# Yelp/nrtsearch

Measured on AMD Instinct MI355X. Metric: queries/sec, 10M-doc 5-term BM25 top-1000, higher is better.
Workload: dtype f32

## Files before the change

### include/nrtgpu_dev.h

```cpp
#ifndef NRTGPU_DEV_H
#define NRTGPU_DEV_H
#include "nrtgpu.h"
#ifdef __cplusplus
extern "C" {
#endif
int  nrtgpu_bench_closed_loop(nrtgpu_ctx* ctx, const nrtgpu_seg* const* segs, const int32_t* doc_bases, int32_t n_segs,
                              const nrtgpu_bm25_query* queries, int32_t n_queries, int32_t clients, int32_t duration_ms,
                              double* out4);
int  nrtgpu_debug_hold_coalescers(nrtgpu_ctx* ctx, int32_t hold);
int  nrtgpu_debug_coalescer_pending(nrtgpu_ctx* ctx, int32_t which);
int  nrtgpu_debug_dist_inject(nrtgpu_ctx* ctx, int32_t step, int32_t failed_query);
int64_t nrtgpu_debug_live_segments(nrtgpu_ctx* ctx);
int  nrtgpu_debug_spec_counters(nrtgpu_ctx* ctx, int64_t* out3);
int  nrtgpu_debug_term_lookup(const nrtgpu_seg* seg, int32_t field_id, int64_t term_hash, int32_t* kind, int32_t* shift, int64_t* bytes);
int  nrtgpu_debug_knn_bounds(int32_t sim, int32_t dim, double q_norm2, double q_l1, float q_absmax, double nv_max, double nv_min,
                             float rows_absmax, float score_boost, double m, double s, double* out10);

#define NRTGPU_FLAG_PROFILE (7 << 8)
int  nrtgpu_get_scan_profile(nrtgpu_ctx* ctx, double* out16);
int  nrtgpu_get_maxscore_profile(nrtgpu_ctx* ctx, double* out16);
int  nrtgpu_debug_maxscore_meetings(nrtgpu_ctx* ctx, int64_t* out4);
int  nrtgpu_debug_wave_kth(const uint64_t* keys, int32_t n, int32_t r, uint64_t* out);
int64_t nrtgpu_get_maxscore_item_walls(nrtgpu_ctx* ctx, uint64_t* out, int64_t cap_slots, int64_t* n_items);

#ifdef __cplusplus
}
#endif
#endif
```

### nrtsearch_amd/_lib.py

```python
from __future__ import annotations

import ctypes as C
import os

_HERE = os.path.dirname(os.path.abspath(__file__))
LIB_PATH = os.environ.get("NRTGPU_LIB_PATH") or os.path.join(_HERE, "libnrtgpu.so")

NRTGPU_OK = 0
NRTGPU_ERR_INVALID_ARG = -1
NRTGPU_ERR_HIP = -2
NRTGPU_ERR_OOM = -3
NRTGPU_ERR_UNSUPPORTED = -4
NRTGPU_ERR_STATE = -5
NRTGPU_ERR_TIMEOUT = -6
NRTGPU_MAX_K = 1024
NRTGPU_MAX_TERMS = 32
NRTGPU_TILE_DOCS = 1024
NRTGPU_FLAG_NO_PREFETCH = 1
NRTGPU_FLAG_NO_FIXED_POINT = 2
NRTGPU_FLAG_NO_MASK_VARIANT = 4
NRTGPU_FLAG_NO_LIVE_FOLD = 8
NRTGPU_FLAG_NO_PRUNE = 16
NRTGPU_FLAG_PACKED_POSTINGS = 32
NRTGPU_FLAG_BLOCKING_WAIT = 64
NRTGPU_FLAG_NO_VECTOR_SKETCH = 128
NRTGPU_FLAG_PROFILE = 7 << 8
NRTGPU_MAX_MASKS = 8

ABI_SYMBOLS = [
    "nrtgpu_version", "nrtgpu_last_error", "nrtgpu_create", "nrtgpu_destroy",
    "nrtgpu_segment_begin", "nrtgpu_segment_add_field_norms", "nrtgpu_segment_add_terms",
    "nrtgpu_segment_add_vectors", "nrtgpu_segment_seal", "nrtgpu_segment_set_live_docs",
    "nrtgpu_segment_set_mask", "nrtgpu_segment_release", "nrtgpu_segment_device_bytes",
    "nrtgpu_search_bm25", "nrtgpu_search_bm25_batch", "nrtgpu_search_bm25_batch_device",
    "nrtgpu_search_bm25_batch_device_epoch", "nrtgpu_exchange_open", "nrtgpu_exchange_close",
    "nrtgpu_search_bm25_coalesced", "nrtgpu_set_coalescing", "nrtgpu_query_supported",
    "nrtgpu_merge_topk_device", "nrtgpu_knn_exact", "nrtgpu_knn_exact_coalesced", "nrtgpu_knn_search", "nrtgpu_rescore_vectors", "nrtgpu_search_hybrid_batch",
    "nrtgpu_int_to_byte4", "nrtgpu_byte4_to_int", "nrtgpu_bm25_idf", "nrtgpu_bm25_avgdl",
    "nrtgpu_bm25_norm_cache", "nrtgpu_slices", "nrtgpu_plan_item_counts", "nrtgpu_fixed_point_scale", "nrtgpu_get_stats", "nrtgpu_reset_stats",
    "nrtgpu_set_slicing",
    "nrtgpu_blend", "nrtgpu_dist_unique_id", "nrtgpu_dist_init", "nrtgpu_dist_search_bm25_batch", "nrtgpu_dist_allgather_merge", "nrtgpu_segment_fork",
    "nrtgpu_search_bm25_batch_device_begin", "nrtgpu_pending_wait", "nrtgpu_set_thread_deadline_ns", "nrtgpu_monotonic_ns", "nrtgpu_last_diagnostics", "nrtgpu_dist_close", "nrtgpu_dist_owned_range", "nrtgpu_dist_search_bm25_batch_mode", "nrtgpu_dist_exchange_merge", "nrtgpu_dist_exchange_merge_checked", "nrtgpu_search_bm25_shard_device_begin", "nrtgpu_note_shard_speculation", "nrtgpu_dist_knn_exact", "nrtgpu_dist_search_hybrid_batch",
    "nrtgpu_knn_exact_relation", "nrtgpu_set_speculation", "nrtgpu_set_shard_share", "nrtgpu_set_thread_slices",
    "nrtgpu_segment_add_byte_vectors", "nrtgpu_knn_exact_bytes", "nrtgpu_knn_search_bytes", "nrtgpu_byte_vector_score",
    "nrtgpu_rescore_byte_vectors", "nrtgpu_search_hybrid_bytes_batch", "nrtgpu_set_knn_gather",
]
DEV_SYMBOLS = [
    "nrtgpu_bench_closed_loop", "nrtgpu_debug_hold_coalescers", "nrtgpu_debug_coalescer_pending", "nrtgpu_debug_live_segments",
    "nrtgpu_debug_spec_counters", "nrtgpu_get_scan_profile", "nrtgpu_get_maxscore_profile", "nrtgpu_get_maxscore_item_walls",
    "nrtgpu_debug_dist_inject", "nrtgpu_debug_term_lookup", "nrtgpu_debug_knn_bounds",
    "nrtgpu_debug_maxscore_meetings", "nrtgpu_debug_wave_kth",
]
DEV_LIB_PATH = os.path.join(_HERE, "libnrtgpu_dev.so")


class Config(C.Structure):
    _fields_ = [("device_id", C.c_int32), ("max_batch", C.c_int32), ("target_items", C.c_int32),
                ("collect_timing", C.c_int32), ("flags", C.c_int32), ("host_threads", C.c_int32),
                ("lookup_budget_pct", C.c_int32), ("reserved", C.c_int32)]


class Term(C.Structure):
    _fields_ = [("field_id", C.c_int32), ("cache_slot", C.c_int32), ("term_hash", C.c_int64),
                ("weight", C.c_float), ("occur", C.c_int32)]


class Bm25Query(C.Structure):
    _fields_ = [("n_terms", C.c_int32), ("terms", C.POINTER(Term)), ("n_caches", C.c_int32),
                ("norm_cache", C.POINTER(C.c_float)), ("k", C.c_int32), ("total_hits_threshold", C.c_int32),
                ("has_after", C.c_int32), ("after_doc", C.c_int32), ("after_score", C.c_float),
                ("min_should_match", C.c_int32), ("min_competitive_score", C.c_float), ("filter_mask", C.c_int32),
                ("must_not_mask", C.c_int32), ("disjunction_max", C.c_int32),
                ("n_more_filters", C.c_int32), ("more_filters", C.POINTER(C.c_int32)),
                ("n_more_must_not", C.c_int32), ("more_must_not", C.POINTER(C.c_int32)),
                ("tie_breaker", C.c_float), ("reserved", C.c_int32)]


class TopDocs(C.Structure):
    _fields_ = [("n_hits", C.c_int32), ("capacity", C.c_int32), ("docs", C.POINTER(C.c_int32)),
                ("scores", C.POINTER(C.c_float)), ("total_hits", C.c_int64),
                ("total_hits_is_lower_bound", C.c_int32)]


class Diagnostics(C.Structure):
    _fields_ = [("total_ms", C.c_double), ("plan_ms", C.c_double), ("queue_ms", C.c_double), ("device_ms", C.c_double),
                ("postings", C.c_int64), ("queries", C.c_int32), ("items_maxscore", C.c_int32), ("items_scan", C.c_int32),
                ("reserved", C.c_int32)]


class Stats(C.Structure):
    _fields_ = [("batches", C.c_int64), ("queries", C.c_int64), ("scan_launches", C.c_int64),
                ("scan_ms", C.c_double), ("scan_postings", C.c_int64), ("scan_items", C.c_int64),
                ("merge_ms", C.c_double), ("host_plan_ms", C.c_double), ("fixed_point_launches", C.c_int64),
                ("maxscore_launches", C.c_int64), ("maxscore_ms", C.c_double), ("maxscore_postings", C.c_int64),
                ("maxscore_items", C.c_int64), ("knn_panels", C.c_int64), ("knn_score_launches", C.c_int64),
                ("knn_score_ms", C.c_double), ("knn_rows", C.c_int64), ("knn_second_passes", C.c_int64), ("knn_sketch_launches", C.c_int64),
                ("spec_queries", C.c_int64), ("spec_reruns", C.c_int64), ("spec_disabled", C.c_int64), ("spec_scattered", C.c_int64)]


class NrtGpuError(RuntimeError):
    def __init__(self, code: int, message: str):
        super().__init__(f"nrtgpu error {code}: {message}")
        self.code = code


_lib = None
_dev = None


def load() -> C.CDLL:
    global _lib
    if _lib is None:
        _lib = _open(LIB_PATH)
    return _lib


def load_dev() -> C.CDLL:
    global _dev
    if _dev is None:
        _dev = _open(DEV_LIB_PATH)
    return _dev


def _open(path: str) -> C.CDLL:
    if not os.path.exists(path):
        raise ImportError(
            f"{path} is missing: build it with `python -m nrtsearch_amd.build` "
            "(hipcc, gfx950). There is no Python/CPU fallback for the query path.")
    L = C.CDLL(path)
    vp, i32, i64, f32 = C.c_void_p, C.c_int32, C.c_int64, C.c_float
    L.nrtgpu_version.restype = C.c_char_p
    L.nrtgpu_last_error.restype = C.c_char_p
    L.nrtgpu_create.argtypes = [C.POINTER(Config), C.POINTER(vp)]
    L.nrtgpu_destroy.argtypes = [vp]
    L.nrtgpu_destroy.restype = None
    L.nrtgpu_segment_begin.argtypes = [vp, i32, i32, C.POINTER(vp)]
    L.nrtgpu_segment_add_field_norms.argtypes = [vp, i32, vp]
    L.nrtgpu_segment_add_terms.argtypes = [vp, i32, i64, vp, vp, vp, vp]
    L.nrtgpu_segment_add_vectors.argtypes = [vp, i32, i32, i32, vp, vp]
    L.nrtgpu_segment_seal.argtypes = [vp]
    L.nrtgpu_segment_set_live_docs.argtypes = [vp, vp, i32]
    L.nrtgpu_segment_set_mask.argtypes = [vp, i32, vp, i32]
    L.nrtgpu_segment_release.argtypes = [vp]
    L.nrtgpu_segment_release.restype = None
    L.nrtgpu_segment_device_bytes.argtypes = [vp]
    L.nrtgpu_segment_device_bytes.restype = i64
    L.nrtgpu_search_bm25.argtypes = [vp, vp, vp, i32, C.POINTER(Bm25Query), C.POINTER(TopDocs)]
    L.nrtgpu_search_bm25_batch.argtypes = [vp, vp, vp, i32, C.POINTER(Bm25Query), i32, C.POINTER(TopDocs)]
    L.nrtgpu_search_bm25_batch_device.argtypes = [vp, vp, vp, i32, C.POINTER(Bm25Query), i32, i32, vp, vp, vp]
    L.nrtgpu_search_bm25_batch_device_epoch.argtypes = [vp, vp, vp, i32, C.POINTER(Bm25Query), i32, i32, vp, vp, vp, i64]
    L.nrtgpu_search_bm25_coalesced.argtypes = [vp, vp, vp, i32, C.POINTER(Bm25Query), C.POINTER(TopDocs)]
    L.nrtgpu_set_coalescing.argtypes = [vp, i32]
    if hasattr(L, "nrtgpu_bench_closed_loop"):
        L.nrtgpu_bench_closed_loop.argtypes = [vp, vp, vp, i32, C.POINTER(Bm25Query), i32, i32, i32, vp]
    L.nrtgpu_query_supported.argtypes = [vp, vp, i32, C.POINTER(Bm25Query)]
    L.nrtgpu_exchange_open.argtypes = [vp, C.c_char_p, i32, i32]
    L.nrtgpu_exchange_close.argtypes = [vp]
    L.nrtgpu_exchange_close.restype = None
    L.nrtgpu_merge_topk_device.argtypes = [vp, i32, i32, i32, vp, vp, vp, vp, vp, C.POINTER(TopDocs)]
    L.nrtgpu_knn_exact.argtypes = [vp, vp, vp, i32, i32, i32, vp, i32, i32, i32, f32, C.POINTER(TopDocs)]
    L.nrtgpu_knn_exact_coalesced.argtypes = [vp, vp, vp, i32, i32, i32, vp, i32, i32, f32, C.POINTER(TopDocs)]
    L.nrtgpu_knn_exact_coalesced.restype = i32
    L.nrtgpu_knn_search.argtypes = [vp, vp, vp, i32, i32, i32, vp, i32, i32, i32, f32, i32, f32, C.POINTER(TopDocs)]
    L.nrtgpu_segment_add_byte_vectors.argtypes = [vp, i32, i32, i32, vp, vp]
    L.nrtgpu_knn_exact_bytes.argtypes = [vp, vp, vp, i32, i32, i32, vp, i32, i32, i32, f32, C.POINTER(TopDocs)]
    L.nrtgpu_knn_search_bytes.argtypes = [vp, vp, vp, i32, i32, i32, vp, i32, i32, i32, f32, i32, f32, C.POINTER(TopDocs)]
    L.nrtgpu_byte_vector_score.argtypes = [i32, i32, i32, i32, i32, vp]
    L.nrtgpu_set_knn_gather.argtypes = [vp, i32]
    L.nrtgpu_rescore_vectors.argtypes = [vp, vp, vp, i32, i32, i32, vp, i32, f32, vp, vp, i32, C.c_double, C.c_double, i32,
                                         C.POINTER(TopDocs)]
    L.nrtgpu_search_hybrid_batch.argtypes = [vp, vp, vp, i32, C.POINTER(Bm25Query), i32, i32, i32, vp, i32, f32,
                                             C.c_double, C.c_double, i32, C.POINTER(TopDocs)]
    L.nrtgpu_rescore_byte_vectors.argtypes = L.nrtgpu_rescore_vectors.argtypes
    L.nrtgpu_search_hybrid_bytes_batch.argtypes = L.nrtgpu_search_hybrid_batch.argtypes
    L.nrtgpu_int_to_byte4.argtypes = [i32]
    L.nrtgpu_byte4_to_int.argtypes = [i32]
    L.nrtgpu_bm25_idf.argtypes = [i64, i64]
    L.nrtgpu_bm25_idf.restype = f32
    L.nrtgpu_bm25_avgdl.argtypes = [i64, i64]
    L.nrtgpu_bm25_avgdl.restype = f32
    L.nrtgpu_bm25_norm_cache.argtypes = [f32, f32, f32, vp]
    L.nrtgpu_bm25_norm_cache.restype = None
    L.nrtgpu_plan_item_counts.argtypes = [i32, vp, i32, vp]
    L.nrtgpu_fixed_point_scale.argtypes = [f32, vp, i32, vp]
    L.nrtgpu_slices.argtypes = [i32, vp, vp, vp, i32, i32, i32, vp, vp]
    L.nrtgpu_get_stats.argtypes = [vp, C.POINTER(Stats)]
    L.nrtgpu_reset_stats.argtypes = [vp]
    L.nrtgpu_set_thread_slices.argtypes = [vp, i32]
    L.nrtgpu_set_speculation.argtypes = [vp, C.c_float]
    L.nrtgpu_set_speculation.restype = C.c_int
    L.nrtgpu_set_shard_share.argtypes = [vp, C.c_int64, C.c_int64]
    L.nrtgpu_set_shard_share.restype = C.c_int
    L.nrtgpu_knn_exact_relation.argtypes = [vp, vp, vp, C.c_int32, C.c_int32, C.c_int32, C.c_int32]
    L.nrtgpu_reset_stats.restype = None
    if hasattr(L, "nrtgpu_debug_hold_coalescers"):
        L.nrtgpu_debug_hold_coalescers.argtypes = [vp, C.c_int32]
        L.nrtgpu_debug_live_segments.argtypes = [vp]
        L.nrtgpu_debug_live_segments.restype = C.c_int64
        L.nrtgpu_debug_spec_counters.argtypes = [vp, vp]
        L.nrtgpu_debug_spec_counters.restype = C.c_int
        L.nrtgpu_get_maxscore_item_walls.argtypes = [vp, vp, C.c_int64, C.POINTER(C.c_int64)]
        L.nrtgpu_get_maxscore_item_walls.restype = C.c_int64
        L.nrtgpu_debug_coalescer_pending.argtypes = [vp, C.c_int32]
        L.nrtgpu_debug_dist_inject.argtypes = [vp, C.c_int32, C.c_int32]
        L.nrtgpu_get_scan_profile.argtypes = [vp, vp]
        L.nrtgpu_get_maxscore_profile.argtypes = [vp, vp]
        L.nrtgpu_debug_term_lookup.argtypes = [vp, i32, i64, C.POINTER(i32), C.POINTER(i32), C.POINTER(i64)]
    if hasattr(L, "nrtgpu_debug_maxscore_meetings"):
        L.nrtgpu_debug_maxscore_meetings.argtypes = [vp, vp]
        L.nrtgpu_debug_wave_kth.argtypes = [vp, i32, i32, vp]
    if hasattr(L, "nrtgpu_debug_knn_bounds"):
        L.nrtgpu_debug_knn_bounds.argtypes = [i32, i32, C.c_double, C.c_double, f32, C.c_double, C.c_double, f32, f32, C.c_double, C.c_double, vp]
    L.nrtgpu_set_slicing.argtypes = [vp, i32, i32, i32]
    L.nrtgpu_blend.argtypes = [i32, vp, vp, vp, vp, i32, i32, i32, i32, C.POINTER(TopDocs)]
    L.nrtgpu_dist_unique_id.argtypes = [vp]
    L.nrtgpu_dist_init.argtypes = [vp, i32, i32, vp]
    L.nrtgpu_dist_search_bm25_batch.argtypes = [vp, vp, vp, i32, C.POINTER(Bm25Query), i32, C.POINTER(TopDocs)]
    L.nrtgpu_dist_allgather_merge.argtypes = [vp, i32, i32, vp, vp, vp, vp, vp, C.POINTER(TopDocs)]
    L.nrtgpu_segment_fork.argtypes = [vp, vp, i32, C.POINTER(vp)]
    L.nrtgpu_search_bm25_batch_device_begin.argtypes = [vp, vp, vp, i32, C.POINTER(Bm25Query), i32, i32, vp, vp, vp, C.c_int64, vp]
    L.nrtgpu_pending_wait.argtypes = [vp]
    L.nrtgpu_set_thread_deadline_ns.argtypes = [C.c_int64]
    L.nrtgpu_set_thread_deadline_ns.restype = None
    L.nrtgpu_monotonic_ns.argtypes = []
    L.nrtgpu_monotonic_ns.restype = C.c_int64
    L.nrtgpu_last_diagnostics.argtypes = [vp]
    L.nrtgpu_dist_owned_range.argtypes = [vp, i32, i32, vp, vp]
    L.nrtgpu_dist_search_bm25_batch_mode.argtypes = [vp, vp, vp, i32, C.POINTER(Bm25Query), i32, i32, C.POINTER(TopDocs)]
    L.nrtgpu_dist_exchange_merge.argtypes = [vp, i32, i32, vp, vp, vp, vp, vp, i32, C.POINTER(TopDocs)]
    L.nrtgpu_dist_exchange_merge_checked.argtypes = [vp, i32, i32, vp, vp, vp, vp, vp, vp, i32, C.POINTER(TopDocs), vp, vp]
    L.nrtgpu_search_bm25_shard_device_begin.argtypes = [vp, vp, vp, i32, C.POINTER(Bm25Query), i32, i32, vp, vp, vp, i32, vp, vp]
    L.nrtgpu_note_shard_speculation.argtypes = [vp, vp, i32, i32, i32]
    L.nrtgpu_dist_knn_exact.argtypes = [vp, vp, vp, i32, i32, i32, vp, i32, i32, i32, C.c_float, i32, C.POINTER(TopDocs)]
    L.nrtgpu_dist_search_hybrid_batch.argtypes = [vp, vp, vp, i32, C.POINTER(Bm25Query), i32, i32, i32, vp, i32, C.c_float, C.c_double, C.c_double,
                                                  i32, i32, C.POINTER(TopDocs)]
    L.nrtgpu_dist_close.argtypes = [vp]
    L.nrtgpu_dist_close.restype = None
    return L


def check(rc: int) -> None:
    if rc != NRTGPU_OK:
        raise NrtGpuError(rc, load().nrtgpu_last_error().decode("utf-8", "replace"))
```

### nrtsearch_amd/api.py

```python
from __future__ import annotations

import ctypes as C
import dataclasses
import os
import threading
from typing import Dict, List, Optional, Sequence, Tuple, Union

import numpy as np

from . import _lib
from ._lib import NrtGpuError

INT_MAX = 2**31 - 1
TOTAL_HITS_THRESHOLD = 1000


EXCHANGE_ALLGATHER, EXCHANGE_ALLTOALL = 0, 1
EXCHANGE_NO_SPECULATION = 0x100


@dataclasses.dataclass(frozen=True)
class TermQuery:
    field: int
    term: int
# ... 441 lines not shown
    def __init__(self, ctx: GpuContext, leaves: Sequence[GpuSegment], stats: IndexStatistics,
                 similarity: Optional[BM25Similarity] = None):
        self.ctx, self.leaves, self.stats = ctx, list(leaves), stats
        self.similarity = similarity or BM25Similarity()
        n = len(self.leaves)
        self._segs = (C.c_void_p * max(n, 1))(*[l._h for l in self.leaves])
        self._bases = (C.c_int32 * max(n, 1))(*[l.doc_base for l in self.leaves])
        self._cache_memo: Dict[int, np.ndarray] = {}

    def _norm_cache(self, field: int) -> np.ndarray:
        c = self._cache_memo.get(field)
        if c is None:
            c = self.similarity.norm_cache(self.stats.fields[field])
            self._cache_memo[field] = c
        return c

    def _marshal(self, queries: Sequence[Query], managers: Sequence[TopScoreDocCollectorManager]) -> _Marshalled:
        m = _Marshalled(len(queries))
        for qi, (query, mgr) in enumerate(zip(queries, managers)):
            clauses, msm, filters, must_nots, dis_max, tie_breaker = _flatten(query)
            fields: List[int] = []
            terms = (_lib.Term * len(clauses))()
            for ti, (field, term, boost, occur) in enumerate(clauses):
                if field not in self.stats.fields:
                    raise UnsupportedQuery(f"no statistics for field {field}")
                if field not in fields:
                    fields.append(field)
                df = self.stats.doc_freq.get((field, term), 0)
                cs = self.stats.fields[field]
                w = np.float32(np.float32(boost) * self.similarity.idf(df, cs.doc_count)) if df > 0 else np.float32(0)
                terms[ti] = _lib.Term(field, fields.index(field), term, float(w), int(occur))
            cache = np.concatenate([self._norm_cache(f) for f in fields]).astype(np.float32)
            m.keep += [terms, cache]
            q = m.queries[qi]
            q.n_terms = len(clauses)
            q.terms = terms
            q.n_caches = len(fields)
            q.norm_cache = cache.ctypes.data_as(C.POINTER(C.c_float))
            q.k = int(mgr.num_hits)
            q.total_hits_threshold = int(mgr.total_hits_threshold)
            q.has_after = int(mgr.after is not None)
            q.after_doc = int(mgr.after.doc) if mgr.after is not None else 0
            q.after_score = float(mgr.after.score) if mgr.after is not None else 0.0
            q.min_should_match = int(msm)
            q.min_competitive_score = float(mgr.min_competitive_score)
            q.filter_mask = int(filters[0]) if filters else 0
            q.must_not_mask = int(must_nots[0]) if must_nots else 0
            q.disjunction_max = int(dis_max)
            q.tie_breaker = float(np.float32(tie_breaker))
            for ids, n_name, p_name in ((filters[1:], "n_more_filters", "more_filters"), (must_nots[1:], "n_more_must_not", "more_must_not")):
                if ids:
                    arr = (C.c_int32 * len(ids))(*[int(x) for x in ids])
                    m.keep.append(arr)
                    setattr(q, n_name, len(ids))
                    setattr(q, p_name, arr)
        return m

    def search_batch(self, queries: Sequence[Query], managers: Sequence[TopScoreDocCollectorManager]) -> List[TopDocs]:
        n = len(queries)
        m = self._marshal(queries, managers)
        outs = (_lib.TopDocs * n)()
        bufs = []
        for qi, mgr in enumerate(managers):
            cap = max(int(mgr.num_hits), 1)
            d = np.zeros(cap, dtype=np.int32)
            s = np.zeros(cap, dtype=np.float32)
            bufs.append((d, s))
            outs[qi].capacity = cap
            outs[qi].docs = d.ctypes.data_as(C.POINTER(C.c_int32))
            outs[qi].scores = s.ctypes.data_as(C.POINTER(C.c_float))
        _lib.check(_lib.load().nrtgpu_search_bm25_batch(self.ctx._h, self._segs, self._bases, len(self.leaves),
                                                        m.queries, n, outs))
        res = []
        for qi in range(n):
            nh = outs[qi].n_hits
            d, s = bufs[qi]
            res.append(TopDocs(d[:nh].copy(), s[:nh].copy(), int(outs[qi].total_hits),
                               bool(outs[qi].total_hits_is_lower_bound)))
        return res

    def search(self, query: Query, manager: TopScoreDocCollectorManager) -> TopDocs:
        return self.search_batch([query], [manager])[0]

    def dist_search_batch(self, queries: Sequence[Query], managers: Sequence[TopScoreDocCollectorManager],
                          mode: int = EXCHANGE_ALLGATHER) -> List[Optional[TopDocs]]:
        n = len(queries)
        m = self._marshal(queries, managers)
        outs = (_lib.TopDocs * n)()
        bufs = []
        for qi, mgr in enumerate(managers):
            cap = max(int(mgr.num_hits), 1)
            d = np.zeros(cap, dtype=np.int32)
            s = np.zeros(cap, dtype=np.float32)
            bufs.append((d, s))
            outs[qi].capacity = cap
            outs[qi].docs = d.ctypes.data_as(C.POINTER(C.c_int32))
            outs[qi].scores = s.ctypes.data_as(C.POINTER(C.c_float))
        _lib.check(_lib.load().nrtgpu_dist_search_bm25_batch_mode(self.ctx._h, self._segs, self._bases, len(self.leaves), m.queries, n,
                                                                  int(mode), outs))
        return [None if outs[qi].total_hits < 0 else
                TopDocs(bufs[qi][0][: outs[qi].n_hits].copy(), bufs[qi][1][: outs[qi].n_hits].copy(), int(outs[qi].total_hits),
                        bool(outs[qi].total_hits_is_lower_bound)) for qi in range(n)]

    def dist_knn_exact(self, field: int, similarity: str, queries: np.ndarray, k: int, boost: float = 1.0,
                       mode: int = EXCHANGE_ALLGATHER) -> List[Optional[TopDocs]]:
        queries = np.ascontiguousarray(np.atleast_2d(queries), dtype=np.float32)
        if similarity == "normalized_cosine":
            queries = np.ascontiguousarray(queries / np.linalg.norm(queries, axis=1, keepdims=True).astype(np.float32), dtype=np.float32)
        nq, dim = queries.shape
        outs, docs, scores = _topdocs_outputs(nq, int(k))
        _lib.check(_lib.load().nrtgpu_dist_knn_exact(self.ctx._h, self._segs, self._bases, len(self.leaves), int(field),
                                                     self.SIMILARITY[similarity], queries.ctypes.data, nq, dim, int(k),
                                                     C.c_float(boost), int(mode), outs))
        return _topdocs_lists(outs, docs, scores, nq, none_if_negative=True)

    def supported(self, query: Query, manager: TopScoreDocCollectorManager) -> bool:
        m = self._marshal([query], [manager])
        rc = _lib.load().nrtgpu_query_supported(self.ctx._h, self._segs, len(self.leaves), m.queries)
        if rc == _lib.NRTGPU_OK:
            return True
        if rc == _lib.NRTGPU_ERR_UNSUPPORTED:
            return False
        _lib.check(rc)
        return False

    def search_coalesced(self, query: Query, manager: TopScoreDocCollectorManager) -> TopDocs:
        m = self._marshal([query], [manager])
        cap = max(int(manager.num_hits), 1)
        d = np.zeros(cap, dtype=np.int32)
        s = np.zeros(cap, dtype=np.float32)
        out = _lib.TopDocs()
        out.capacity = cap
        out.docs = d.ctypes.data_as(C.POINTER(C.c_int32))
        out.scores = s.ctypes.data_as(C.POINTER(C.c_float))
        _lib.check(_lib.load().nrtgpu_search_bm25_coalesced(self.ctx._h, self._segs, self._bases, len(self.leaves),
                                                            m.queries, C.byref(out)))
        return TopDocs(d[: out.n_hits].copy(), s[: out.n_hits].copy(), int(out.total_hits), bool(out.total_hits_is_lower_bound))

    SIMILARITY = {"cosine": 0, "dot_product": 1, "normalized_cosine": 1, "l2_norm": 2, "max_inner_product": 3}

    def knn_exact(self, field: int, similarity: str, queries: np.ndarray, k: int, boost: float = 1.0) -> List[TopDocs]:
        queries = np.ascontiguousarray(np.atleast_2d(queries), dtype=np.float32)
        if similarity == "normalized_cosine":
            queries = queries / np.linalg.norm(queries, axis=1, keepdims=True).astype(np.float32)
            queries = np.ascontiguousarray(queries, dtype=np.float32)
        nq, dim = queries.shape
        outs, docs, scores = _topdocs_outputs(nq, int(k))
        _lib.check(_lib.load().nrtgpu_knn_exact(self.ctx._h, self._segs, self._bases, len(self.leaves), int(field),
                                                self.SIMILARITY[similarity], queries.ctypes.data, nq, dim, int(k),
                                                C.c_float(boost), outs))
        return _topdocs_lists(outs, docs, scores, nq)

    def knn_exact_coalesced(self, field: int, similarity: str, query: np.ndarray, k: int, boost: float = 1.0) -> TopDocs:
        query = np.ascontiguousarray(query, dtype=np.float32).reshape(-1)
        if similarity == "normalized_cosine":
            query = np.ascontiguousarray(query / np.linalg.norm(query).astype(np.float32), dtype=np.float32)
        out = _lib.TopDocs()
        docs = np.zeros(k, dtype=np.int32)
        scores = np.zeros(k, dtype=np.float32)
        out.capacity = k
        out.docs = docs.ctypes.data_as(C.POINTER(C.c_int32))
        out.scores = scores.ctypes.data_as(C.POINTER(C.c_float))
        _lib.check(_lib.load().nrtgpu_knn_exact_coalesced(self.ctx._h, self._segs, self._bases, len(self.leaves), int(field),
                                                          self.SIMILARITY[similarity], query.ctypes.data, int(query.shape[0]), int(k),
                                                          C.c_float(boost), C.byref(out)))
        return TopDocs(docs[: out.n_hits].copy(), scores[: out.n_hits].copy(), int(out.total_hits), bool(out.total_hits_is_lower_bound))
# ... 198 lines not shown
        self.scores = np.zeros((self.n, kmax), dtype=np.float32)
        for qi in range(self.n):
            self._outs[qi].capacity = kmax
            self._outs[qi].docs = self.docs[qi].ctypes.data_as(C.POINTER(C.c_int32))
            self._outs[qi].scores = self.scores[qi].ctypes.data_as(C.POINTER(C.c_float))

    def run(self, d_keys: int, d_counts: int, d_hits: int) -> None:
        _lib.check(_lib.load().nrtgpu_merge_topk_device(
            self.ctx._h, self.n_lists, self.n, self.k_stride, C.c_void_p(d_keys), C.c_void_p(d_counts),
            C.c_void_p(d_hits), self._ks.ctypes.data, self._thr.ctypes.data, self._outs))

    def run_dist(self, d_keys: int, d_counts: int, d_hits: int, mode: int = EXCHANGE_ALLGATHER) -> None:
        _lib.check(_lib.load().nrtgpu_dist_exchange_merge(
            self.ctx._h, self.n, self.k_stride, C.c_void_p(d_keys), C.c_void_p(d_counts), C.c_void_p(d_hits),
            self._ks.ctypes.data, self._thr.ctypes.data, int(mode), self._outs))

    def run_dist_checked(self, d_keys: int, d_counts: int, d_hits: int, d_guess: int, mode: int = EXCHANGE_ALLGATHER) -> np.ndarray:
        failed = np.zeros(self.n, dtype=np.uint8)
        n_failed = C.c_int32(0)
        _lib.check(_lib.load().nrtgpu_dist_exchange_merge_checked(
            self.ctx._h, self.n, self.k_stride, C.c_void_p(d_keys), C.c_void_p(d_counts), C.c_void_p(d_hits), C.c_void_p(d_guess),
            self._ks.ctypes.data, self._thr.ctypes.data, int(mode), self._outs, failed.ctypes.data, C.byref(n_failed)))
        return np.flatnonzero(failed) if n_failed.value else np.zeros(0, dtype=np.int64)

    def kth_keys(self) -> np.ndarray:
        n_hits = np.frombuffer(self._outs, dtype=np.int32).reshape(self.n, C.sizeof(_lib.TopDocs) // 4)[:, 0]
        rows = np.arange(self.n)
        col = self._ks.astype(np.int64) - 1
        keys = (self.scores.view(np.uint32)[rows, col].astype(np.uint64) << np.uint64(32)) | (np.uint64(0xFFFFFFFF) - self.docs[rows, col].astype(np.uint64))
        return np.where(n_hits >= self._ks, keys, np.uint64(0))

    def owned(self, qi: int) -> bool:
        return self._outs[qi].total_hits >= 0

    def topdocs(self, qi: int) -> TopDocs:
        o = self._outs[qi]
        return TopDocs(self.docs[qi, : o.n_hits].copy(), self.scores[qi, : o.n_hits].copy(), int(o.total_hits),
                       bool(o.total_hits_is_lower_bound))


def merge_topk_device(ctx: GpuContext, n_lists: int, n_queries: int, k_stride: int, d_keys: int, d_counts: int,
                      d_hits: int, ks: Sequence[int], thresholds: Sequence[int]) -> List[TopDocs]:
    pm = PreparedMerge(ctx, n_lists, n_queries, k_stride, ks, thresholds)
    pm.run(d_keys, d_counts, d_hits)
    return [pm.topdocs(qi) for qi in range(n_queries)]


def slices(max_docs: Sequence[int], num_docs: Optional[Sequence[int]] = None, virtual_shards: int = 1,
           slice_max_docs: int = 250_000, slice_max_segments: int = 5):
    n = len(max_docs)
    md = np.ascontiguousarray(max_docs, dtype=np.int32)
    nd = np.ascontiguousarray(num_docs if num_docs is not None else max_docs, dtype=np.int32)
    sl = np.full(max(n, 1), -1, dtype=np.int32)
    sh = np.full(max(n, 1), -1, dtype=np.int32)
    ns = _lib.load().nrtgpu_slices(n, md.ctypes.data, nd.ctypes.data, None, int(virtual_shards), int(slice_max_docs),
                                   int(slice_max_segments), sl.ctypes.data, sh.ctypes.data)
    if ns < 0:
        _lib.check(ns)
    out: List[List[int]] = [[] for _ in range(ns)]
    for i in range(n):
        out[sl[i]].append(i)
    return out, sh[:n].tolist()


def debug_knn_bounds(sim: int, dim: int, q_norm2: float, q_l1: float, q_absmax: float, nv_max: float, nv_min: float,
                     rows_absmax: float, score_boost: float = 1.0, m: float = 0.0, s: float = 0.0) -> dict:
    out = np.zeros(10, dtype=np.float64)
    _lib.check(_lib.load().nrtgpu_debug_knn_bounds(int(sim), int(dim), float(q_norm2), float(q_l1), C.c_float(q_absmax), float(nv_max),
                                                   float(nv_min), C.c_float(rows_absmax), C.c_float(score_boost), float(m), float(s),
                                                   out.ctypes.data))
    names = ("e32", "e16", "result_upper32", "result_upper16", "estimate_lower32", "estimate_lower16", "q_scale", "rows_scale")
    d = {n: float(out[i]) for i, n in enumerate(names)}
    d["q_scale_usable"], d["rows_scale_usable"] = bool(out[8]), bool(out[9])
    return d


def debug_wave_kth(keys: np.ndarray, r: int) -> int:
    keys = np.ascontiguousarray(keys, dtype=np.uint64)
    out = np.zeros(1, dtype=np.uint64)
    _lib.check(_lib.load().nrtgpu_debug_wave_kth(keys.ctypes.data, len(keys), int(r), out.ctypes.data))
    return int(out[0])


def blend(retriever_docs: Sequence[np.ndarray], retriever_scores: Optional[Sequence[np.ndarray]] = None,
          boosts: Optional[Sequence[float]] = None, mode: str = "rrf", k: int = 60, start_hit: int = 0, top_hits: int = 10) -> TopDocs:
    n = len(retriever_docs)
    docs = [np.ascontiguousarray(d, dtype=np.int32) for d in retriever_docs]
    scs = [np.ascontiguousarray(s_, dtype=np.float32) for s_ in retriever_scores] if retriever_scores is not None else None
    dp = (C.c_void_p * max(n, 1))(*[d.ctypes.data for d in docs])
    sp = (C.c_void_p * max(n, 1))(*[s_.ctypes.data for s_ in scs]) if scs is not None else None
    counts = np.asarray([len(d) for d in docs], dtype=np.int32)
    b = np.ascontiguousarray(boosts, dtype=np.float32) if boosts is not None else None
    cap = max(int(top_hits), 1)
    od, os_ = np.zeros(cap, np.int32), np.zeros(cap, np.float32)
    out = _lib.TopDocs()
    out.capacity = cap
    out.docs = od.ctypes.data_as(C.POINTER(C.c_int32))
    out.scores = os_.ctypes.data_as(C.POINTER(C.c_float))
    _lib.check(_lib.load().nrtgpu_blend(n, dp, sp, counts.ctypes.data, b.ctypes.data if b is not None else None,
                                        0 if mode == "rrf" else 1, int(k), int(start_hit), int(top_hits), C.byref(out)))
    return TopDocs(od[: out.n_hits].copy(), os_[: out.n_hits].copy(), int(out.total_hits), bool(out.total_hits_is_lower_bound))


def weighted_rrf_blend(retriever_hits: Sequence[np.ndarray], boosts: Optional[Sequence[float]] = None, k: int = 60,
                       start_hit: int = 0, top_hits: int = 10) -> TopDocs:
    if k < 1:
        raise ValueError(f"k must be >= 1, got: {k}")
    if top_hits == 0 or start_hit > top_hits:
        return TopDocs(np.zeros(0, np.int32), np.zeros(0, np.float32), 0, True)
    merged: Dict[int, np.float32] = {}
    for ri, docs in enumerate(retriever_hits):
        w = np.float32(1.0 if boosts is None else boosts[ri])
        for i, doc in enumerate(np.asarray(docs).tolist()):
            contrib = np.float32(w / np.float32(k + i + 1))
            merged[doc] = np.float32(merged[doc] + contrib) if doc in merged else contrib
    order = sorted(merged.items(), key=lambda kv: (-float(kv[1]), kv[0]))[: min(top_hits, len(merged))]
    page = order[min(start_hit, len(order)):]
    return TopDocs(np.asarray([d for d, _ in page], np.int32), np.asarray([s for _, s in page], np.float32),
                   len(merged), True)
```

### nrtsearch_amd/csrc/devtools.cpp

```cpp
#include "runtime_internal.h"
#include "../../include/nrtgpu_dev.h"

extern "C" int nrtgpu_bench_closed_loop(nrtgpu_ctx* ctx, const nrtgpu_seg* const* segs, const int32_t* doc_bases,
                                        int32_t n_segs, const nrtgpu_bm25_query* queries, int32_t n_queries,
                                        int32_t clients, int32_t duration_ms, double* out4) {
  if (!ctx || !queries || !out4 || n_queries <= 0 || clients <= 0 || duration_ms <= 0)
    return fail(NRTGPU_ERR_INVALID_ARG, "bad closed-loop arguments");
  std::vector<std::vector<float>> lat((size_t)clients);
  std::vector<int> rcs((size_t)clients, 0);
  std::vector<std::string> errs((size_t)clients);
  const auto t_begin = std::chrono::steady_clock::now();
  const auto t_stop = t_begin + std::chrono::milliseconds(duration_ms);
  auto client = [&](int c) {
    int32_t kmax = 1;
    for (int i = 0; i < n_queries; ++i) kmax = std::max(kmax, queries[i].k);
    std::vector<int32_t> docs((size_t)kmax);
    std::vector<float> scores((size_t)kmax);
    size_t i = (size_t)c * 7919u;
    for (;;) {
      const auto t0 = std::chrono::steady_clock::now();
      if (t0 >= t_stop) break;
      nrtgpu_topdocs o{};
      o.capacity = kmax;
      o.docs = docs.data();
      o.scores = scores.data();
      const int rc = nrtgpu_search_bm25_coalesced(ctx, segs, doc_bases, n_segs, &queries[i % (size_t)n_queries], &o);
      if (rc != 0) {
        rcs[(size_t)c] = rc;
        errs[(size_t)c] = g_last_error;
        break;
      }
      lat[(size_t)c].push_back(std::chrono::duration<float, std::milli>(std::chrono::steady_clock::now() - t0).count());
      ++i;
    }
  };
  std::vector<std::thread> pool;
  for (int c = 0; c < clients; ++c) pool.emplace_back(client, c);
  for (auto& t : pool) t.join();
  const double secs = std::chrono::duration<double>(std::chrono::steady_clock::now() - t_begin).count();
  for (int c = 0; c < clients; ++c)
    if (rcs[(size_t)c] != 0) return fail(rcs[(size_t)c], "client %d: %s", c, errs[(size_t)c].c_str());
  std::vector<float> all;
  for (auto& v : lat) all.insert(all.end(), v.begin(), v.end());
  std::sort(all.begin(), all.end());
  out4[0] = (double)all.size();
  out4[1] = secs;
  out4[2] = all.empty() ? 0.0 : all[all.size() / 2];
  out4[3] = all.empty() ? 0.0 : all[(size_t)((double)all.size() * 0.99)];
  return NRTGPU_OK;
}


extern "C" int nrtgpu_debug_knn_bounds(int32_t sim, int32_t dim, double q_norm2, double q_l1, float q_absmax, double nv_max, double nv_min,
                                       float rows_absmax, float score_boost, double m, double s, double* out10) {
  if (!out10 || sim < 0 || sim > 3 || dim <= 0 || (dim & 15)) return fail(NRTGPU_ERR_INVALID_ARG, "bad knn_bounds arguments");
  float q_scale = 1.0f, rows_scale = 1.0f;
  const bool q_ok = hostmath::knn_sketch_scale(q_absmax, &q_scale), rows_ok = hostmath::knn_sketch_scale(rows_absmax, &rows_scale);
  const double e_rel = (double)hostmath::knn_e_rel(), b = (double)score_boost;
  const float e32 = hostmath::knn_bound32(sim, dim, q_norm2, nv_max, b);
  const float e16 = hostmath::knn_bound16(sim, dim, q_norm2, q_l1, 1.0 / (double)q_scale, nv_max, nv_min, 1.0 / (double)rows_scale, b);
  out10[0] = (double)e32;
  out10[1] = (double)e16;
  out10[2] = knn_result_upper(sim, m, (double)e32, e_rel, b);
  out10[3] = knn_result_upper(sim, m, (double)e16, e_rel, b);
  out10[4] = knn_estimate_lower(sim, s, (double)e32, e_rel, b);
  out10[5] = knn_estimate_lower(sim, s, (double)e16, e_rel, b);
  out10[6] = (double)q_scale;
  out10[7] = (double)rows_scale;
  out10[8] = q_ok ? 1.0 : 0.0;
  out10[9] = rows_ok ? 1.0 : 0.0;
  return NRTGPU_OK;
}

extern "C" int nrtgpu_debug_maxscore_meetings(nrtgpu_ctx* ctx, int64_t* out4) {
  if (!ctx || !out4) return fail(NRTGPU_ERR_INVALID_ARG, "NULL argument");
  std::lock_guard<std::mutex> lk(ctx->stats_mu);
  for (int i = 0; i < 4; ++i) out4[i] = ctx->ms_meetings[i];
  return NRTGPU_OK;
}

extern "C" int nrtgpu_debug_wave_kth(const uint64_t* keys, int32_t n, int32_t r, uint64_t* out) {
  if (!keys || !out || n < 1 || n > kMsCandCap || r < 1 || r > n) return fail(NRTGPU_ERR_INVALID_ARG, "bad wave_kth arguments (1 <= r <= n <= %d)", kMsCandCap);
  uint64_t* d = nullptr;
  if (hipMalloc((void**)&d, ((size_t)n + 1) * sizeof(uint64_t)) != hipSuccess) return fail(NRTGPU_ERR_OOM, "hipMalloc");
  hipError_t e = hipMemcpy(d, keys, (size_t)n * sizeof(uint64_t), hipMemcpyHostToDevice);
  if (e == hipSuccess) {
    launch_debug_wave_kth(nullptr, d, (uint32_t)n, (uint32_t)r, d + n);
    e = hipGetLastError();
  }
  if (e == hipSuccess) e = hipMemcpy(out, d + n, sizeof(uint64_t), hipMemcpyDeviceToHost);
  (void)hipFree(d);
  if (e != hipSuccess) return fail(NRTGPU_ERR_HIP, "wave_kth: %s", hipGetErrorString(e));
  return NRTGPU_OK;
}
```

### nrtsearch_amd/csrc/kernels.hip

```cpp
#include <hip/hip_runtime.h>
#include <stdint.h>

#include "bm25_common.hiph"

namespace nrtgpu {

struct ScanSmem {
  uint64_t acc[kScanWaves][kTileDocs];
  uint64_t cand[kCandCap];
  uint32_t tab[kTabTerms][kTabEntries];
  float    cache[kLdsCaches][256];
  alignas(16) uint32_t w_incl[kScanWaves][kMaxTerms];
  alignas(16) uint32_t w_rec[kScanWaves][kMaxTerms][4];
  uint32_t w_before[kScanWaves][kMaxTerms];
  TopkScratch sc;
  uint64_t theta;
  uint64_t thr;
  uint32_t cnt;
  uint32_t tile_cand;
  uint32_t slot_hits[kSliceSlots];
  uint32_t slot_slice[kSliceSlots];
  uint32_t rz_flag;
  uint32_t cnt_valid;
  uint32_t next_tile;
// ... 848 lines not shown
  }
}

__global__ __launch_bounds__(256)
void apply_live_kernel(const uint32_t* __restrict__ docids, uint32_t* __restrict__ fnorm, uint64_t n,
                       const uint64_t* __restrict__ live) {
  const uint64_t stride = (uint64_t)gridDim.x * blockDim.x;
  for (uint64_t p = (uint64_t)blockIdx.x * blockDim.x + threadIdx.x; p < n; p += stride) {
    uint32_t c = fnorm[p];
    const bool esc = (c >> 31) != 0u;
    if (esc) c &= ~0x40000000u;
    else if ((c >> 20) != 0u) c = (((c >> 20) & 15u) << 9) | (c & 0x1FCu);
    bool is_live = true;
    if (live) {
      const uint32_t d = docids[p];
      is_live = (live[d >> 6] >> (d & 63u)) & 1ull;
    }
    if (!is_live) c = esc ? (c | 0x40000000u) : ((((c >> 9) & 15u) << 20) | (c & 0x1FCu));
    fnorm[p] = c;
  }
}

__global__ __launch_bounds__(256)
void pack_count_kernel(const uint32_t* __restrict__ fnorm, uint64_t n, uint32_t* __restrict__ counts) {
  __shared__ uint32_t total;
  if (threadIdx.x == 0) total = 0;
  __syncthreads();
  const uint64_t p0 = (uint64_t)blockIdx.x << kPackEscBlockShift;
  uint32_t mine = 0;
  for (uint32_t i = threadIdx.x; i < (1u << kPackEscBlockShift); i += 256u) {
    const uint64_t p = p0 + i;
    if (p < n && (fnorm[p] >> 31) != 0u) ++mine;
  }
  if (mine) atomicAdd(&total, mine);
  __syncthreads();
  if (threadIdx.x == 0) counts[blockIdx.x] = total;
}

__global__ __launch_bounds__(256)
void pack_write_kernel(const uint32_t* __restrict__ docids, const uint32_t* __restrict__ fnorm, uint64_t n,
                       const uint32_t* __restrict__ dir, uint32_t* __restrict__ exceptions, uint32_t* __restrict__ packed) {
  __shared__ uint32_t wave_cnt[8][4];
  const uint32_t lane = threadIdx.x & 63u, wave = threadIdx.x >> 6;
  const uint64_t p0 = (uint64_t)blockIdx.x << kPackEscBlockShift;
  uint32_t c[8];
  unsigned long long ball[8];
#pragma unroll
  for (int r = 0; r < 8; ++r) {
    const uint64_t p = p0 + (uint64_t)r * 256u + threadIdx.x;
    c[r] = p < n ? fnorm[p] : 0u;
    ball[r] = __builtin_amdgcn_ballot_w64((c[r] >> 31) != 0u);
    if (lane == 0) wave_cnt[r][wave] = (uint32_t)__popcll(ball[r]);
  }
  __syncthreads();
  const uint32_t e_block = dir[blockIdx.x];
#pragma unroll
  for (int r = 0; r < 8; ++r) {
    const uint64_t p = p0 + (uint64_t)r * 256u + threadIdx.x;
    if (p >= n) continue;
    uint32_t code = c[r] >> 2;
    if ((c[r] >> 31) != 0u) {
      uint32_t before = 0;
      for (int rr = 0; rr < 8; ++rr)
        for (int ww = 0; ww < 4; ++ww)
          if (rr < r || (rr == r && (uint32_t)ww < wave)) before += wave_cnt[rr][ww];
      const uint32_t e = e_block + before + (uint32_t)__popcll(ball[r] & ((1ull << lane) - 1ull));
      exceptions[e] = c[r];
      code = kPackEscBase + (e & kPackEscLowMask);
    }
    packed[p] = ((docids[p] & kPackDocMask) << kPackCodeBits) | code;
  }
}

__global__ __launch_bounds__(256)
void expand_terms_kernel(const DQExpand* __restrict__ qx, const DQTerm* __restrict__ qterms, const uint32_t* __restrict__ out_begin,
                         uint32_t n_queries, uint32_t n_leaves, DTerm* __restrict__ out) {
  const uint32_t i = blockIdx.x * blockDim.x + threadIdx.x;
  if (i >= n_queries * n_leaves) return;
  const uint32_t ob = out_begin[i];
  if (ob == 0xFFFFFFFFu) return;
  const uint32_t q = i / n_leaves, leaf = i - q * n_leaves;
  const DQExpand x = qx[q];
  const DQTerm* const qt = qterms + x.term_begin;
  for (uint32_t t = 0; t < x.n_terms; ++t) {
    DTerm d = qt[t].table[leaf];
    if (d.docids == nullptr) continue;
    const uint32_t cnt = __float_as_uint(d.weight);
    const float w = qt[t].weight;
    uint32_t rank = 0;
    for (uint32_t u = 0; u < x.n_terms; ++u) {
      if (u == t) continue;
      const DTerm& o = qt[u].table[leaf];
      if (o.docids == nullptr) continue;
      const uint32_t oc = __float_as_uint(o.weight);
      const float ow = qt[u].weight;
      const bool before = x.by_weight ? (ow > w || (ow == w && (oc < cnt || (oc == cnt && u < t))))
                                      : (oc > cnt || (oc == cnt && u < t));
      rank += before ? 1u : 0u;
    }
    d.weight = w;
    d.cache_slot = qt[t].cache_slot;
    d.tab_slot = qt[t].tab_slot;
    d.fx_scale = qt[t].fx_scale;
    d.fx_shift = qt[t].fx_shift;
    out[ob + rank] = d;
  }
}
void launch_expand_terms(hipStream_t stream, const DQExpand* qx, const DQTerm* qterms, const uint32_t* out_begin, uint32_t n_queries,
                         uint32_t n_leaves, DTerm* out) {
  const uint64_t n = (uint64_t)n_queries * n_leaves;
  if (n == 0) return;
  hipLaunchKernelGGL(expand_terms_kernel, dim3((uint32_t)((n + 255) / 256)), dim3(256), 0, stream, qx, qterms, out_begin, n_queries,
                     n_leaves, out);
}

__global__ __launch_bounds__(256)
void slice_relation_kernel(const uint32_t* __restrict__ slice_sum, const DQuery* __restrict__ queries, uint32_t n_slices,
                           uint64_t* __restrict__ out_hits, uint32_t n) {
  const uint32_t q = blockIdx.x * blockDim.x + threadIdx.x;
  if (q >= n) return;
  if ((out_hits[q] >> 48) != 0ull) return;
  const uint32_t floor_ = queries[q].gte_floor;
  if (floor_ == 0xFFFFFFFFu) return;
  const uint32_t* sums = slice_sum + queries[q].slice_base;
  bool gte = false;
  for (uint32_t i = 0; i < n_slices; ++i) gte = gte || sums[i] > floor_;
  if (gte) out_hits[q] += kHitsPrunedUnit;
}
void launch_slice_relation(hipStream_t stream, const uint32_t* slice_sum, const DQuery* queries, uint32_t n_slices, uint64_t* out_hits,
                           uint32_t n) {
  if (n == 0) return;
  hipLaunchKernelGGL(slice_relation_kernel, dim3((n + 255) / 256), dim3(256), 0, stream, slice_sum, queries, n_slices, out_hits, n);
}

__global__ __launch_bounds__(256)
void patch_hits_kernel(const uint64_t* __restrict__ lower, uint64_t* __restrict__ hits, uint32_t n) {
  const uint32_t q = blockIdx.x * blockDim.x + threadIdx.x;
  if (q < n && lower[q] != 0ull && (hits[q] >> 48) != 0ull) hits[q] = kHitsPrunedUnit + lower[q] + (hits[q] & kHitsSpecInvalid);
}
void launch_patch_hits(hipStream_t stream, const uint64_t* lower, uint64_t* hits, uint32_t n) {
  if (n == 0) return;
  hipLaunchKernelGGL(patch_hits_kernel, dim3((n + 255) / 256), dim3(256), 0, stream, lower, hits, n);
}

void launch_pack_count(hipStream_t stream, const uint32_t* fnorm, uint64_t n, uint32_t n_blocks, uint32_t* counts) {
  if (n_blocks == 0) return;
  hipLaunchKernelGGL(pack_count_kernel, dim3(n_blocks), dim3(256), 0, stream, fnorm, n, counts);
}
void launch_pack_write(hipStream_t stream, const uint32_t* docids, const uint32_t* fnorm, uint64_t n, uint32_t n_blocks,
                       const uint32_t* dir, uint32_t* exceptions, uint32_t* packed) {
  if (n_blocks == 0) return;
  hipLaunchKernelGGL(pack_write_kernel, dim3(n_blocks), dim3(256), 0, stream, docids, fnorm, n, dir, exceptions, packed);
}
void launch_apply_live(hipStream_t stream, const uint32_t* docids, uint32_t* fnorm, uint64_t n, const uint64_t* live) {
  if (n == 0) return;
  const uint64_t blocks = (n + 1023) / 1024;
  hipLaunchKernelGGL(apply_live_kernel, dim3((uint32_t)(blocks < 8192 ? blocks : 8192)), dim3(256), 0, stream, docids, fnorm, n, live);
}
void launch_bm25_scan(hipStream_t stream, bool fixed_point, bool pipelined, bool packed, int ablation, uint32_t n_items, const DItem* items,
                      const DPart* parts, const DTerm* terms, const DQuery* queries, const float* caches, unsigned long long* theta_g,
                      unsigned long long* quant_g, const DExchange* xch, uint32_t* slice_sum, uint64_t* item_keys, uint32_t* item_counts,
                      uint64_t* item_hits, uint32_t k_stride, uint64_t* item_prof) {
  if (n_items == 0) return;
#define NRT_LAUNCH_K(F, P, A, K)                                                                                  \
  hipLaunchKernelGGL((bm25_scan_kernel<F, P, A, K>), dim3(n_items), dim3(kScanThreads), 0, stream, items, parts, terms, queries, \
                     caches, theta_g, quant_g, xch, slice_sum, item_keys, item_counts, item_hits, k_stride, item_prof)
#define NRT_LAUNCH(F, P, A)                 \
  do {                                      \
    if (packed) NRT_LAUNCH_K(F, P, A, true);  \
    else NRT_LAUNCH_K(F, P, A, false);      \
  } while (0)
#define NRT_LAUNCH_FX(P, A)            \
  do {                                 \
    if (fixed_point) NRT_LAUNCH(true, P, A); \
    else NRT_LAUNCH(false, P, A);      \
  } while (0)
  if (ablation == 8) { NRT_LAUNCH(true, true, 8); return; }
  if (ablation == 9) { NRT_LAUNCH_FX(true, 9); return; }
  if (!pipelined) { NRT_LAUNCH_FX(false, 0); return; }
  switch (ablation) {
#ifdef NRTGPU_DEV
    case 1: NRT_LAUNCH_K(false, true, 1, false); break;
    case 2: NRT_LAUNCH_K(false, true, 2, false); break;
    case 3: NRT_LAUNCH_K(false, true, 3, false); break;
    case 4: NRT_LAUNCH_K(false, true, 4, false); break;
    case 6: NRT_LAUNCH_K(false, true, 6, false); break;
    case 7: NRT_LAUNCH_FX(true, 7); break;
#endif
    default: NRT_LAUNCH_FX(true, 0); break;
  }
#undef NRT_LAUNCH_FX
#undef NRT_LAUNCH
#undef NRT_LAUNCH_K
}

void launch_merge_topk(hipStream_t stream, uint32_t n_queries, const uint64_t* in_keys, const uint32_t* in_counts,
                       const uint64_t* in_hits, const uint32_t* list_idx, const uint32_t* q_base,
// ... 19 lines not shown
```

### nrtsearch_amd/csrc/maxscore.hip

```cpp
#include <hip/hip_runtime.h>
#include <stdint.h>

#include "bm25_common.hiph"

namespace nrtgpu {

constexpr int kMsWinWords = kMsWinDocs / 32;
constexpr int kSl = kMsSlots;
typedef uint32_t u32x2 __attribute__((ext_vector_type(2)));
typedef const NRT_GLOBAL u32x2* gvec2_ptr;

struct alignas(16) WClause {
  uint64_t docids, fnorm;
  uint64_t begin;
  uint32_t count, pad0;
  float    weight;
  int32_t  fx_scale;
  uint32_t flags;
  uint32_t pad;
  uint64_t u_after;
  uint64_t look;
  uint64_t cells, start;
};
static_assert(sizeof(WClause) == 80, "WClause layout");
// ... 144 lines not shown
    if (guess > s.theta) {
      s.theta = guess;
      s.thr = acc_threshold<true>(guess, fx_E);
      atomicMax(theta_g, (unsigned long long)guess);
      atomicMax(s.spec_slot, (unsigned long long)guess);
    }
    const uint32_t ws = s.wins_started;
    s.spec_at = ws >= s.q_wins ? 0u : max(ws * s.spec_grow16 / 16u, ws + (uint32_t)kMsWaves);
  }
  __syncthreads();
  if (tid == 0) s.rz_flag = 0;
  __syncthreads();
}

__device__ __forceinline__ bool ms_meet(MsSmem& s, uint32_t k, int fx_E, unsigned long long* theta_g, const DExchange* xch = nullptr,
                                        uint32_t query = 0) {
  __syncthreads();
  if (!__hip_atomic_load(&s.rz_flag, __ATOMIC_RELAXED, __HIP_MEMORY_SCOPE_WORKGROUP)) return false;
  ms_compact((__attribute__((address_space(3))) MsSmem*)&s, k, fx_E, theta_g, xch, query);
  return true;
}

__device__ __noinline__ void ms_estimate(__attribute__((address_space(3))) MsSmem* sp, uint32_t k, int fx_E,
                                         unsigned long long* theta_g, const DExchange* xch) {
  MsSmem& s = *(MsSmem*)sp;
  const uint32_t lane = threadIdx.x & 63u;
  const uint32_t ws = (uint32_t)__builtin_amdgcn_readfirstlane((int)__hip_atomic_load(&s.wins_started, __ATOMIC_RELAXED, __HIP_MEMORY_SCOPE_WORKGROUP));
  const uint32_t at = (uint32_t)__builtin_amdgcn_readfirstlane((int)__hip_atomic_load(&s.spec_at, __ATOMIC_RELAXED, __HIP_MEMORY_SCOPE_WORKGROUP));
  const uint32_t n = (uint32_t)__builtin_amdgcn_readfirstlane((int)__hip_atomic_load(&s.cnt, __ATOMIC_RELAXED, __HIP_MEMORY_SCOPE_WORKGROUP));
  if (at != 0u && ws >= at && n <= (uint32_t)kMsCandCap) {
    const bool exchanging = xch && xch->world > 1u;
    uint32_t r = 0;
    if (s.spec_z16 != 0u && !exchanging && __hip_atomic_load(&s.prune_on, __ATOMIC_RELAXED, __HIP_MEMORY_SCOPE_WORKGROUP) != 0u) {
      const float m = (float)k * fminf(1.0f, (float)ws / (float)max(s.q_wins, 1u));
      const float rr = m + (float)s.spec_z16 * (1.0f / 16.0f) * sqrtf(m) + 2.0f;
      r = rr < (float)k ? (uint32_t)rr : 0u;
    }
    uint64_t guess = 0;
    if (r != 0u && n > r) guess = topk_kth_wave(s.cand, n, r, &s.sc);
    if (lane == 0u) {
      if (guess > s.theta) {
        __hip_atomic_store(&s.theta, guess, __ATOMIC_RELAXED, __HIP_MEMORY_SCOPE_WORKGROUP);
        __hip_atomic_store(&s.thr, acc_threshold<true>(guess, fx_E), __ATOMIC_RELAXED, __HIP_MEMORY_SCOPE_WORKGROUP);
        atomicMax(theta_g, (unsigned long long)guess);
        atomicMax(s.spec_slot, (unsigned long long)guess);
      }
      s.spec_at = ws >= s.q_wins ? 0u : max(ws * s.spec_grow16 / 16u, ws + (uint32_t)kMsWaves);
      s.n_est += 1u;
    }
  }
  wave_lds_phase();
  if (lane == 0u) __hip_atomic_store(&s.spec_busy, 0u, __ATOMIC_RELEASE, __HIP_MEMORY_SCOPE_WORKGROUP);
}

__device__ __forceinline__ bool ms_reserve(MsSmem& s, uint32_t lane, uint32_t mine, uint32_t& pos) {
  const uint32_t incl = scan64_dpp(mine);
  const uint32_t wave_total = (uint32_t)__builtin_amdgcn_readlane((int)incl, 63);
  uint32_t wbase = 0;
  if (lane == 0) {
    wbase = atomicAdd(&s.cnt, wave_total);
    if (wbase + wave_total > (uint32_t)kMsCandCap) {
      if (wbase <= (uint32_t)kMsCandCap) s.cnt_valid = wbase;
      __hip_atomic_store(&s.rz_flag, 1u, __ATOMIC_RELAXED, __HIP_MEMORY_SCOPE_WORKGROUP);
    }
  }
  wbase = (uint32_t)__builtin_amdgcn_readfirstlane((int)wbase);
  pos = wbase + incl - mine;
  return wbase + wave_total <= (uint32_t)kMsCandCap;
}

template <bool PROF, bool PACKED, int SHAPES>
__global__ __launch_bounds__(kMsThreads)
void bm25_maxscore_kernel(const MsArgs* __restrict__ launch) {
  constexpr bool TWO = SHAPES == 2;
  __shared__ MsSmem s;
  const uint32_t tid = threadIdx.x;
  const uint32_t wave = tid >> 6, lane = tid & 63u;
  for (uint32_t round = 0;; ++round) {
    const uint64_t wall_entry = PROF ? wall_clock64() : 0ull;
    const ms_args_ptr ap = ms_fresh(launch);
    const __attribute__((address_space(4))) DHelp& hp = ap->help;
    const DItem* const items = as_global(ap->items);
    const DPart* const parts = as_global(ap->parts);
    const DTerm* const terms = as_global(ap->terms);
    const DExchange* const xch = as_global(ap->xch);
    bool helper = false;
    uint32_t my_item = 0, out_slot = 0;
    {
      const uint32_t min_rem = hp.min_rem & 0xFFFFu;
      const bool greedy = ((hp.min_rem >> 16) & 1u) != 0u;
      for (int attempt = 0; attempt < 2; ++attempt) {
        if (tid == 0) {
          s.pick = 0ull;
          s.role[0] = __hip_atomic_load(hp.item_next, __ATOMIC_RELAXED, __HIP_MEMORY_SCOPE_AGENT);
          s.role[1] = __hip_atomic_load(hp.help_used, __ATOMIC_RELAXED, __HIP_MEMORY_SCOPE_AGENT);
          s.role[2] = 0u;
          s.role[3] = __hip_atomic_load(hp.help_off, __ATOMIC_RELAXED, __HIP_MEMORY_SCOPE_AGENT);
        }
        __syncthreads();
        const uint32_t q_next = s.role[0];
        const bool queue_empty = attempt == 1 || q_next >= hp.n_own;
        const bool slots_left = s.role[1] < hp.n_help;
        if (queue_empty && (!slots_left || s.role[3] != 0u)) return;
        const bool look = slots_left && (queue_empty || (hp.alpha16 != 0u && q_next >= hp.n_cus + hp.n_cus / 4u));
        if (look) {
          const uint64_t now = wall_clock64();
          float t_rem = 0.f;
          if (!queue_empty) {
            uint32_t mine = 0;
            for (uint32_t i = tid; i < hp.n_own; i += kMsThreads) {
              const uint64_t t0 = __hip_atomic_load(hp.item_t0 + i, __ATOMIC_RELAXED, __HIP_MEMORY_SCOPE_AGENT);
              if (t0 == 0ull) continue;
              mine += min(items[i].flags >> 8, (uint32_t)kMsWaves + __hip_atomic_load(hp.win_next + i, __ATOMIC_RELAXED, __HIP_MEMORY_SCOPE_AGENT));
            }
            mine = (uint32_t)__builtin_amdgcn_readlane((int)scan64_dpp(mine), 63);
            if (lane == 0 && mine != 0u) atomicAdd(&s.role[2], mine);
            __syncthreads();
            const uint32_t handed = s.role[2];
            const uint64_t ts = __hip_atomic_load(hp.t_start, __ATOMIC_RELAXED, __HIP_MEMORY_SCOPE_AGENT);
            t_rem = (handed == 0u || ts == 0ull || now <= ts) ? 3.0e38f
                    : (float)(now - ts) * (float)(hp.total_wins > handed ? hp.total_wins - handed : 0u) / (float)handed * ((float)hp.alpha16 * (1.0f / 16.0f));
          }
          for (uint32_t i = tid; i < hp.n_own; i += kMsThreads) {
            const uint32_t fl = items[i].flags;
            if ((fl & 3u) == kMsModeExact) continue;
            const uint32_t nw = fl >> 8;
            const uint32_t taken = (uint32_t)kMsWaves + __hip_atomic_load(hp.win_next + i, __ATOMIC_RELAXED, __HIP_MEMORY_SCOPE_AGENT);
            if (taken + min_rem > nw) continue;
            const uint64_t t0 = __hip_atomic_load(hp.item_t0 + i, __ATOMIC_RELAXED, __HIP_MEMORY_SCOPE_AGENT);
            if (t0 == 0ull || now <= t0) continue;
            const uint32_t hc = __hip_atomic_load(hp.help_cnt + i, __ATOMIC_RELAXED, __HIP_MEMORY_SCOPE_AGENT);
            const float left = (float)(now - t0) * (float)(nw - taken) / ((float)(taken - (uint32_t)kMsWaves + 1u) * (float)(1u + hc));
            if (!queue_empty && !(left > t_rem)) continue;
            uint32_t hsh = ((blockIdx.x + round * gridDim.x) * 0x9E3779B9u) ^ (i * 0x85EBCA6Bu) ^ (uint32_t)now;
            hsh ^= hsh >> 16; hsh *= 0x7FEB352Du; hsh ^= hsh >> 15; hsh *= 0x846CA68Bu; hsh ^= hsh >> 16;
            const float u = ((float)(hsh >> 8) + 0.5f) * (1.0f / 16777216.0f);
            const float key = greedy ? left : left / -__logf(u);
            atomicMax((unsigned long long*)&s.pick, ((unsigned long long)__float_as_uint(key) << 32) | (unsigned long long)(i + 1u));
          }
        }
        __syncthreads();
        if (tid == 0) {
          const uint64_t pick = s.pick;
          uint32_t r_item = 0xFFFFFFFFu, r_slot = 0xFFFFFFFFu;
          if ((uint32_t)pick != 0u) {
            const uint32_t slot = atomicAdd(hp.help_used, 1u);
            if (slot < hp.n_help) {
              r_slot = slot;
              r_item = (uint32_t)pick - 1u;
              atomicAdd(hp.help_cnt + r_item, 1u);
            }
          } else if (queue_empty && look) {
            __hip_atomic_store(hp.help_off, 1u, __ATOMIC_RELAXED, __HIP_MEMORY_SCOPE_AGENT);
          }
          if (r_slot == 0xFFFFFFFFu && !queue_empty) {
            const uint32_t it = atomicAdd(hp.item_next, 1u);
            if (it < hp.n_own) r_item = it;
          }
          s.role[0] = r_item;
          s.role[1] = r_slot;
        }
        __syncthreads();
        const uint32_t r_item = s.role[0], r_slot = s.role[1];
        __syncthreads();
        if (r_item != 0xFFFFFFFFu) {
          my_item = r_item;
          helper = r_slot != 0xFFFFFFFFu;
// ... 32 lines not shown
      const uint64_t theta0 = __hip_atomic_load(my_theta_g, __ATOMIC_RELAXED, __HIP_MEMORY_SCOPE_AGENT);
      s.theta = theta0;
      s.thr = acc_threshold<true>(theta0, fx_E);
      s.cnt = 0;
      s.cnt_valid = 0;
      s.rz_flag = 0;
      s.spec_busy = 0;
      s.n_meet = s.n_over = s.n_est = 0;
      if (!helper) {
        const unsigned long long now0 = (unsigned long long)wall_clock64();
        __hip_atomic_store(hp.item_t0 + my_item, now0, __ATOMIC_RELAXED, __HIP_MEMORY_SCOPE_AGENT);
        if (my_item == 0u) __hip_atomic_store(hp.t_start, now0, __ATOMIC_RELAXED, __HIP_MEMORY_SCOPE_AGENT);
      }
      s.prune_on = mode == kMsModePrune ? 1u : 0u;
      const bool spec = hp.spec_g != nullptr && hp.spec_z16 != 0u;
      s.wins_started = 0;
      s.q_wins = spec ? as_global(ap->q_wins)[item.query] : 0u;
      s.spec_z16 = spec ? hp.spec_z16 : 0u;
      s.spec_slot = spec ? as_global(hp.spec_g) + item.query : nullptr;
      s.spec_at = spec ? max(hp.spec_sched & 255u, 1u) : 0u;
      s.spec_grow16 = max((hp.spec_sched >> 8) & 255u, 17u);
      s.spec_meet = (hp.spec_sched >> 16) & 1u;
      for (int i = 0; i < kSliceSlots; ++i) s.slot_hits[i] = s.slot_slice[i] = 0u;
      for (int i = 0; i < 16; ++i) s.prof[i] = 0;
    }
    const uint64_t t_item0 = PROF ? __builtin_readcyclecounter() : 0ull;
    const uint64_t wall0 = PROF ? wall_clock64() : 0ull;
    uint64_t tc_meet = 0, tc_part = 0, tc_walk = 0;
    __syncthreads();
    if (xch && tid < 64u) {
      const uint64_t pb = exchange_bound(*xch, item.query, 0ull, tid);
      if (tid == 0 && pb > s.theta) {
        s.theta = pb;
        s.thr = acc_threshold<true>(pb, fx_E);
      }
    }
    for (uint32_t slot = 0; slot < item.n_tabs; ++slot) {
      const float w = items[my_item].tab_weight[slot];
      const int scale = items[my_item].tab_scale[slot];
      const float* cache = &s.cache[items[my_item].tab_cache[slot]][0];
      for (uint32_t e = tid; e < (uint32_t)kTabEntries; e += kMsThreads)
        s.tab[slot][e] = e < (uint32_t)kTabNorms ? 0u : score_value<true>(bm25_score(w, (float)(int32_t)(e >> 7), cache[e & 127u]), scale);
    }
    __syncthreads();
  #ifndef NRT_MS_PHASE_CLOCKS
    if (PROF && tid == 0) s.prof[8] = __builtin_readcyclecounter() - t_item0;
  #endif

    uint32_t* const seen = &s.seen[wave][0];
    WClause* const wcl = &s.wc[wave][0];
    const uint32_t wcl_addr = lds_addr(wcl);
    uint32_t wave_hits = 0;
    uint32_t cur_slot = 0;
    uint64_t pc_post = 0, pc_surv = 0, pc_look = 0, pc_cand = 0, pc_chunks = 0, pc_wins = 0;
  #ifdef NRT_MS_PHASE_CLOCKS
    uint64_t ph[9] = {0, 0, 0, 0, 0, 0, 0, 0, 0}, ph_t = 0;
  #endif
  #ifdef NRT_MS_COUNT_ROUNDS
    uint64_t pc_dense = 0, pc_sparse = 0, pc_steps = 0, pc_tas = 0, pc_crounds = 0;
  #endif
    const uint32_t item_wins = item.flags >> 8;
    uint32_t sc_mul = 1u;
    if (ap->scatter != 0u && item_wins > 3u && item_wins < 65536u) {
      const uint32_t primes[4] = {2654435761u, 2246822519u, 3266489917u, 668265263u};
      uint32_t best = 0xFFFFFFFFu;
  #pragma unroll
      for (int i = 0; i < 4; ++i) {
        const uint32_t a = primes[i] % item_wins;
        const uint32_t x = a * 1000u, y = item_wins * 618u;
        const uint32_t dist = x > y ? x - y : y - x;
        if (a > 1u && dist < best) {
          best = dist;
          sc_mul = a;
        }
      }
    }
    auto window_of_take = [&](uint32_t h) -> uint32_t {
      return (sc_mul == 1u || h >= item_wins) ? h : (h * sc_mul) % item_wins;
    };
    uint32_t g = window_of_take(helper ? (uint32_t)kMsWaves + (uint32_t)__builtin_amdgcn_readfirstlane((int)first_win) : wave);
    uint32_t pi = 0;
    uint32_t win_base = 0;

    for (;;) {
      DPart part;
      uint32_t part_wins = 0;
      if (sc_mul != 1u) {
        pi = 0;
        win_base = 0;
      }
      for (;; ++pi) {
        if (pi >= item.n_parts) break;
        part = parts[item.part_begin + pi];
        part_wins = (part.tile_end - (part.tile_begin & ~(win_tiles - 1u)) + win_tiles - 1u) / win_tiles;
        if (g < win_base + part_wins) break;
        win_base += part_wins;
      }
      if (pi >= item.n_parts) break;
      {
        const uint32_t p_slot = part.slice >> 24;
        if (p_slot != cur_slot && wave_hits != 0u) {
          if (lane == 0) atomicAdd(&s.slot_hits[cur_slot], wave_hits);
          wave_hits = 0;
        }
        cur_slot = p_slot;
        if (lane == 0) s.slot_slice[p_slot] = part.slice & 0xFFFFFFu;
      }
      const uint32_t n_terms = part.n_terms;
      const DTerm* const part_terms = terms + part.term_begin;

      uint64_t my_ub = 0, my_suf = 0;
      const uint64_t t_part0 = PROF ? __builtin_readcyclecounter() : 0ull;
      const DTerm mt = part_terms[min(lane, n_terms - 1u)];
      {
        uint32_t ub_raw = 0;
        for (uint32_t pass = 0; pass * 4u < n_terms; ++pass) {
          const uint32_t tt = pass * 4u + (lane >> 4), i = lane & 15u;
          const DTerm* Tp = part_terms + min(tt, n_terms - 1u);
          const DTermAux* ax = Tp->aux;
          const float w = Tp->weight;
          const int scale = Tp->fx_scale;
          const float* cache = &s.cache[Tp->cache_slot][0];
          uint32_t v = 0;
          if (tt < n_terms) {
            if (i < 12u) {
              const uint32_t nb = ax->min_norm[i];
              if (nb != 0xFFu) v = score_value<true>(bm25_score(w, (float)(int32_t)(i + 1u), cache[nb]), scale);
            } else if (i == 12u) {
              const uint32_t mf = ax->esc_max_freq;
              if (mf != 0u) v = score_value<true>(bm25_score(w, (float)(int32_t)mf, cache[ax->esc_min_norm]), scale);
            }
          }
  #pragma unroll
          for (int dlt = 8; dlt > 0; dlt >>= 1) v = max(v, (uint32_t)__shfl_xor((int)v, dlt, 64));
          const uint32_t got = (uint32_t)__shfl((int)v, (int)((lane & 3u) * 16u), 64);
          if ((lane >> 2) == pass) ub_raw = got;
        }
        if (lane < n_terms) my_ub = (uint64_t)ub_raw << mt.fx_shift;
      }
      uint64_t my_after = 0;
      {
        uint64_t run = 0;
        for (int m = (int)n_terms - 1; m >= 0; --m) {
          const uint64_t ub = readlane_u64(my_ub, (uint32_t)m);
          if (lane == (uint32_t)m) my_after = run;
          run = use_max ? max(run, ub) : run + ub;
          if (lane == (uint32_t)m) my_suf = run;
        }
      }
      const gu32_ptr my_cells = (gu32_ptr)mt.cell_off;
      const uint32_t my_shift = mt.shift;
      if (lane < n_terms) {
        WClause w;
        w.docids = (uint64_t)mt.docids;
        w.fnorm = (uint64_t)mt.fnorm;
        w.begin = 0;
        w.count = w.pad0 = 0;
        w.weight = mt.weight;
        w.fx_scale = mt.fx_scale;
        const DTermAux* const ax = mt.aux;
        const uint32_t look_kind = ax->look_kind;
        w.flags = ((mt.tab_slot & 0xFFFFu) < (uint32_t)kTabTerms ? (mt.tab_slot & 0xFFFFu) : 7u) | (TWO && (mt.tab_slot & kTabSlotRequired) ? 8u : 0u) |
                  (mt.fx_shift << 4) | (mt.cache_slot << 8) | ((mt.shift & 31u) << 16) | ((look_kind & 7u) << 24) | (((uint32_t)ax->look_shift & 31u) << 27);
        w.pad = 0;
        w.u_after = my_after;
        w.look = look_kind != kLookNone ? (uint64_t)ax->look : 0ull;
        w.cells = (uint64_t)mt.cell_off;
        w.start = mt.start;
        wcl[lane] = w;
      }
      const uint32_t req_mask = TWO ? (uint32_t)__builtin_amdgcn_ballot_w64(lane < n_terms && (mt.tab_slot & kTabSlotRequired) != 0u) : 0u;
      const uint32_t first_req = req_mask != 0u ? (uint32_t)__builtin_ctz(req_mask) : 0xFFu;
      if (PROF) tc_part += __builtin_readcyclecounter() - t_part0;

      for (;;) {
        const uint64_t t_win0 = PROF ? __builtin_readcyclecounter() : 0ull;
        const uint32_t ta = (part.tile_begin & ~(win_tiles - 1u)) + (g - win_base) * win_tiles;
        const uint32_t t0 = max(ta, part.tile_begin);
        const uint32_t t1 = min(ta + win_tiles, part.tile_end);
        const uint32_t doc_lo = t0 * (uint32_t)kTileDocs;
        const uint32_t doc_span = min(t1 * (uint32_t)kTileDocs, part.max_doc) - doc_lo;
        if (PROF) pc_wins += 1;
        {
          uint32_t est = 0;
          if (lane == 0) {
            const uint32_t ws = atomicAdd(&s.wins_started, 1u) + 1u, at = s.spec_at;
            if (at != 0u && ws >= at) {
              if (s.spec_meet != 0u) __hip_atomic_store(&s.rz_flag, 1u, __ATOMIC_RELAXED, __HIP_MEMORY_SCOPE_WORKGROUP);
              else est = atomicCAS(&s.spec_busy, 0u, 1u) == 0u ? 1u : 0u;
            }
          }
          if (__builtin_amdgcn_readfirstlane((int)est) != 0)
            ms_estimate((__attribute__((address_space(3))) MsSmem*)&s, k, fx_E, my_theta_g, xch);
        }
        uint32_t g_new = 0;
        if (lane == 0) g_new = (uint32_t)kMsWaves + __hip_atomic_fetch_add(win_next_g, 1u, __ATOMIC_RELAXED, __HIP_MEMORY_SCOPE_AGENT);
        uint64_t theta_other = 0, thr_other = 0;
        if (multi_item) {
          theta_other = __hip_atomic_load(my_theta_g, __ATOMIC_RELAXED, __HIP_MEMORY_SCOPE_AGENT);
          thr_other = acc_threshold<true>(theta_other, fx_E);
          if (mode == kMsModeCount && lane == 0 && __hip_atomic_load(my_prune_g, __ATOMIC_RELAXED, __HIP_MEMORY_SCOPE_AGENT) != 0u)
            __hip_atomic_store(&s.prune_on, 1u, __ATOMIC_RELAXED, __HIP_MEMORY_SCOPE_WORKGROUP);
        }
        uint32_t my_lo = 0, my_hi = 0;
        if (lane < n_terms) {
          my_lo = my_cells[t0 >> my_shift];
          my_hi = my_cells[((t1 - 1u) >> my_shift) + 1u];
        }
        if (n_terms > 1u) {
  #pragma unroll
          for (int j = 0; j < kMsWinWords / 64 / 4; ++j) *(u32x4*)&seen[(lane + 64u * (uint32_t)j) * 4u] = u32x4{0u, 0u, 0u, 0u};
        }
        uint32_t ng = 0;
        {
          const uint64_t thr_w = __hip_atomic_load(&s.prune_on, __ATOMIC_RELAXED, __HIP_MEMORY_SCOPE_WORKGROUP) ? loosen(max(s.thr, thr_other)) : 0ull;
          const uint64_t pb = mt.start + my_lo, pe = mt.start + my_hi;
          if (lane < n_terms) {
            if (my_suf >= thr_w && pe > pb && (!SHAPES || msm <= 1u || lane + msm <= n_terms) && (!TWO || lane <= first_req)) ng = (uint32_t)((pe - (pb & ~3ull) + (uint64_t)(kSl - 1)) / (uint64_t)kSl);
            *(u32x4*)&wcl[lane].begin = u32x4{(uint32_t)pb, (uint32_t)(pb >> 32), (uint32_t)(pe - pb), 0u};
          }
        }
        const uint32_t incl = scan32_dpp(ng);
        uint32_t pre[kMsMaxTerms];
  #pragma unroll
        for (int i = 0; i < kMsMaxTerms; ++i) pre[i] = (uint32_t)__builtin_amdgcn_readlane((int)incl, i);
        const uint32_t n_groups = pre[kMsMaxTerms - 1];

  #ifdef NRT_MS_PHASE_CLOCKS
        if (PROF) ph_t = t_win0;
  #endif
        NRT_PH_MARK(0);
        for (uint32_t v0 = 0; v0 < n_groups; v0 += 64u) {
          const uint32_t v = v0 + lane;
          const bool act = v < n_groups;
          uint32_t c = 0, before = 0;
  #pragma unroll
          for (int i = 0; i < kMsMaxTerms - 1; ++i) {
            c += (v >= pre[i]) ? 1u : 0u;
            before = (v >= pre[i]) ? pre[i] : before;
          }
          const uint32_t c_first = (uint32_t)__builtin_amdgcn_readfirstlane((int)c);
          const uint64_t theta = max(s.theta, theta_other), thr = loosen(max(s.thr, thr_other));
          const bool pruning = __hip_atomic_load(&s.prune_on, __ATOMIC_RELAXED, __HIP_MEMORY_SCOPE_WORKGROUP) != 0u;
          const uint64_t thr_p = pruning ? thr : 0ull;
          if (readlane_u64(my_suf, c_first) < thr_p) break;
          if (PROF) pc_chunks += 1;
          const uint32_t rec = wcl_addr + c * (uint32_t)sizeof(WClause);
          const u32x4 r0 = *(const u32x4*)lds_ptr(rec), r1 = *(const u32x4*)lds_ptr(rec + 16u), r2 = *(const u32x4*)lds_ptr(rec + 32u);
          const uint64_t u_after = *(const uint64_t*)lds_ptr(rec + 48u);
          const uint64_t col_d = ((uint64_t)r0[1] << 32) | r0[0], col_c = ((uint64_t)r0[3] << 32) | r0[2];
          const uint64_t p_begin = ((uint64_t)r1[1] << 32) | r1[0];
          const uint32_t flags = r2[2];
          const uint32_t q0 = (v - before) * (uint32_t)kSl;
          const uint64_t mine0 = (p_begin & ~3ull) + (uint64_t)q0;
          uint32_t d[kSl], cd[kSl];
  #pragma unroll
          for (int j = 0; j < kSl; ++j) d[j] = cd[j] = 0u;
          if (act) {
            const u32x4 d0 = __builtin_nontemporal_load((gvec_ptr)(col_d + mine0 * 4u));
            const u32x4 d1 = kSl > 4 ? __builtin_nontemporal_load((gvec_ptr)(col_d + mine0 * 4u) + 1) : d0;
            if (PACKED) {
              const uint32_t sw = doc_lo & ~kPackDocMask;
  #pragma unroll
              for (int j = 0; j < 4; ++j) {
                d[j] = (d0[j] >> kPackCodeBits) | sw;
                cd[j] = (d0[j] & kPackCodeMask) << 2;
                if (kSl > 4) {
                  d[(4 + j) % kSl] = (d1[j] >> kPackCodeBits) | sw;
                  cd[(4 + j) % kSl] = (d1[j] & kPackCodeMask) << 2;
                }
              }
            } else {
              const u32x4 c0 = __builtin_nontemporal_load((gvec_ptr)(col_c + mine0 * 4u));
              const u32x4 c1 = kSl > 4 ? __builtin_nontemporal_load((gvec_ptr)(col_c + mine0 * 4u) + 1) : c0;
  #pragma unroll
              for (int j = 0; j < 4; ++j) {
                d[j] = d0[j];
                cd[j] = c0[j];
                if (kSl > 4) {
                  d[(4 + j) % kSl] = d1[j];
                  cd[(4 + j) % kSl] = c1[j];
                }
              }
            }
          }
          NRT_PH_MARK(1);
          uint32_t vmask = 0;
          {
            const uint32_t rel = q0 - ((uint32_t)p_begin & 3u), cnt = act ? r1[2] : 0u;
  #pragma unroll
            for (int j = 0; j < kSl; ++j)
              if (rel + (uint32_t)j < cnt && d[j] - doc_lo < doc_span) vmask |= 1u << j;
          }
          uint32_t val[kSl];
          {
            const uint32_t tab = flags & 7u;
            const char* tb = (const char*)&s.tab[tab == 7u ? 0u : tab][0];
            uint32_t cor = 0;
  #pragma unroll
// ... 582 lines not shown
```

### nrtsearch_amd/csrc/plan.h

```cpp
#pragma once
#include <math.h>
#include <stdint.h>

namespace nrtgpu {

#ifndef NRT_SCAN_WAVES
#define NRT_SCAN_WAVES 12
#endif
#ifndef NRT_TILE_DOCS
#define NRT_TILE_DOCS 1024
#endif
constexpr int kTileDocs = NRT_TILE_DOCS;
constexpr int kScanWaves = NRT_SCAN_WAVES;
constexpr int kScanThreads = kScanWaves * 64;
static_assert(kScanWaves % 4 == 0 && kTileDocs % 64 == 0 && kTileDocs / 64 <= 16, "scan workgroup shape");
static_assert(kScanWaves * kTileDocs * 8 <= 96 * 1024, "accumulators exceed their LDS share");
constexpr int kCandCap = (kScanWaves == 12) ? 1920 : 1664;
constexpr int kMergeCap = 2048;
constexpr int kLdsCaches = 4;
constexpr int kTabTerms = 5;
constexpr int kTabMaxFreq = 12;
constexpr int kTabNorms = 128;
constexpr int kTabEntries = (kTabMaxFreq + 1) * kTabNorms;
constexpr int kMaxK = 1024;
constexpr int kMaxTerms = 32;
constexpr uint32_t kPackDocBits = 20;
constexpr uint32_t kPackCodeBits = 12;
constexpr uint32_t kPackCodeMask = (1u << kPackCodeBits) - 1u;
constexpr uint32_t kPackDocMask = (1u << kPackDocBits) - 1u;
constexpr uint32_t kPackEscBase = (uint32_t)kTabEntries;
constexpr uint32_t kPackEscBlockShift = 11;
constexpr uint32_t kPackEscLowMask = (1u << kPackEscBlockShift) - 1u;
static_assert(kPackEscBase + kPackEscLowMask < (1u << kPackCodeBits), "exception codes must fit the 12-bit code");
constexpr uint32_t kPackMaxCellShift = kPackDocBits - 10;
static_assert(kTileDocs == 1024 || kPackMaxCellShift > 0, "packed postings assume 1024-doc sub-tiles");

struct DTermAux;
struct alignas(16) DTerm {
  const uint32_t* docids;
  const uint32_t* fnorm;
  const uint32_t* cell_off;
  uint64_t start;
  const DTermAux* aux;
  uint32_t shift;
  float    weight;
  uint32_t cache_slot;
  uint32_t tab_slot;
  int32_t  fx_scale;
  uint32_t fx_shift;
};
static_assert(sizeof(DTerm) == 64, "DTerm layout");

struct alignas(16) DQTerm {
  const DTerm* table;
  float    weight;
  uint32_t cache_slot;
  uint32_t tab_slot;
  int32_t  fx_scale;
  uint32_t fx_shift;
  uint32_t pad;
};
static_assert(sizeof(DQTerm) == 32, "DQTerm layout");
struct alignas(16) DQExpand {
  uint32_t term_begin;
  uint32_t n_terms;
  uint32_t by_weight;
  uint32_t pad;
};
static_assert(sizeof(DQExpand) == 16, "DQExpand layout");

constexpr uint32_t kLookNone = 0, kLookBits = 1, kLookCells = 2;
struct alignas(16) DTermAux {
  const void* look;
  uint8_t  min_norm[12];
  uint8_t  esc_min_norm;
  uint8_t  look_kind;
  uint8_t  look_shift;
  uint8_t  pad;
  uint32_t esc_max_freq;
  uint32_t pad2;
};
static_assert(sizeof(DTermAux) == 32, "DTermAux layout");

#ifndef NRT_MS_WIN_TILES
#define NRT_MS_WIN_TILES 64
#endif
#ifndef NRT_MS_WAVES
#define NRT_MS_WAVES 12
#endif
#ifndef NRT_MS_SLOTS
#define NRT_MS_SLOTS 8
#endif
constexpr int kMsWaves = NRT_MS_WAVES;
constexpr int kMsSlots = NRT_MS_SLOTS;
static_assert(kMsSlots == 4 || kMsSlots == 8, "MaxScore kernel: 4 or 8 postings per lane");
constexpr int kMsThreads = kMsWaves * 64;
static_assert(kMsThreads <= 1024, "a workgroup holds at most 16 waves");
constexpr int kMsWinTiles = NRT_MS_WIN_TILES;
constexpr int kMsWinDocs = kMsWinTiles * kTileDocs;
constexpr int kMsMaxTerms = 8;
constexpr int64_t kMsExactMaxPostings = 1 << 18;
#ifndef NRT_MS_CAND_CAP
#define NRT_MS_CAND_CAP (NRT_MS_WIN_TILES > 32 ? 2304 : 3072)
#endif
constexpr int kMsCandCap = NRT_MS_CAND_CAP;
static_assert(kMsCandCap >= kMaxK + 512, "candidate buffer too small");
constexpr uint64_t kHitsPrunedUnit = 1ull << 48;
constexpr uint64_t kHitsSpecInvalid = 1ull << 47;

struct alignas(16) DPart {
  const uint64_t* live_bits;
  uint32_t term_begin;
  uint32_t n_terms;
  uint32_t tile_begin, tile_end;
  uint32_t max_doc;
  int32_t  doc_base;
  uint32_t tile_offset;
  uint32_t slice;
};
static_assert(sizeof(DPart) == 48, "DPart layout");

struct alignas(16) DItem {
  uint32_t query;
  uint32_t part_begin;
  uint32_t n_parts;
  uint32_t cache_off;
  uint32_t n_caches;
  uint32_t n_tabs;
  float    tab_weight[kTabTerms];
  uint32_t tab_cache[kTabTerms];
  int32_t  tab_scale[kTabTerms];
  int32_t  fx_E;
  uint32_t peer_slot;
  uint32_t flags;
};
static_assert(sizeof(DItem) == 96, "DItem layout");

struct alignas(16) DQuery {
  uint32_t k;
  uint32_t has_after;
  int32_t  after_doc;
  float    after_score;
  uint32_t item_begin;
  uint32_t n_items;
  uint32_t min_should_match;
  uint32_t combine_max;
  uint32_t gte_floor;
  uint32_t slice_base;
  uint32_t sec_mode;
  float    tie_breaker;
};
static_assert(sizeof(DQuery) == 48, "DQuery layout");
constexpr int kSliceSlots = 8;
constexpr uint32_t kMsModePrune = 0, kMsModeExact = 1, kMsModeCount = 2;
constexpr uint32_t kMsSecNone = 0, kMsSecTieBreaker = 1, kMsSecReqOpt = 2;
constexpr uint32_t kTabSlotNone = 0xFFFFu, kTabSlotRequired = 1u << 16;
constexpr int kMsmCountShift = 56;

struct DHelp {
  uint32_t* win_next;
  uint32_t* help_cnt;
  unsigned long long* item_t0;
  uint32_t* help_head;
  uint32_t* help_query;
  uint32_t* help_off;
  uint32_t* item_next;
  uint32_t* help_used;
  unsigned long long* t_start;
  uint32_t n_own, n_help;
  uint32_t slot_base;
  uint32_t min_rem;
  uint32_t total_wins;
  uint32_t alpha16;
  uint32_t n_cus;
  uint32_t persistent;
  unsigned long long* spec_g;
  uint32_t spec_z16, spec_sched;
  unsigned long long* walls;
};

struct DExchange;
struct MsArgs {
  const DItem* items;
  const DPart* parts;
  const DTerm* terms;
  const DQuery* queries;
  const float* caches;
  unsigned long long* theta_g;
  uint32_t* slice_sum;
  uint32_t* q_prune;
  const DExchange* xch;
  uint64_t* item_keys;
  uint32_t* item_counts;
  uint64_t* item_hits;
  uint64_t* item_prof;
  const uint32_t* q_wins;
  uint32_t k_stride;
  uint32_t scatter;
  DHelp help;
};

constexpr int kExchangeSlots = 8;
struct alignas(16) DExchange {
  unsigned long long* slot;
  uint32_t world, rank;
  uint32_t stride;
  uint32_t tag;
};
static_assert(sizeof(DExchange) == 32, "DExchange layout");

struct DVecSeg {
  const float* vecs;
  const float* vnorm2;
  const int32_t* ord_to_doc;
  int32_t doc_base, max_doc, n_vec, pad;
};
static_assert(sizeof(DVecSeg) == 40, "DVecSeg layout");

struct alignas(16) DKnnLeaf {
  const void* sketch;
  const float* vnorm2;
  const int32_t* ord_to_doc;
  const uint64_t* accept;
  int64_t tile_begin;
  int32_t n_rows, doc_base;
  float inv_rows_scale;
  int32_t pad[3];
};
static_assert(sizeof(DKnnLeaf) == 64, "DKnnLeaf layout");

__host__ __device__ inline double knn_result_upper(int sim, double m, double e_abs, double e_rel, double boost) {
  if (sim == 2) {
    if (!(m > 0.0)) return 0.0;
    const double d2 = boost / m - 1.0;
    const double lo = d2 - (e_abs + e_rel * (1.0 + d2));
    return boost / (1.0 + (lo > 0.0 ? lo : 0.0)) * (1.0 + 1e-6);
  }
  return (m + e_abs + e_rel * (m < 0.0 ? -m : m)) * (1.0 + 1e-6);
}
__host__ __device__ inline double knn_estimate_lower(int sim, double s, double e_abs, double e_rel, double boost) {
  if (sim == 2) {
    if (!(s > 0.0)) return 0.0;
    const double d2 = boost / s - 1.0;
    return boost / (1.0 + (d2 > 0.0 ? d2 : 0.0) + e_abs + e_rel * (1.0 + d2)) * (1.0 - 1e-6);
  }
  return (s - (e_abs + e_rel * (s < 0.0 ? -s : s))) * (1.0 - 1e-6);
}

struct alignas(16) DKnnBytesLeaf {
  const void* tiles;
  const int32_t* vnorm2;
  const int32_t* ord_to_doc;
  const uint64_t* accept;
  int64_t tile_begin;
  int32_t n_rows, doc_base;
  int32_t pad[4];
};
static_assert(sizeof(DKnnBytesLeaf) == 64, "DKnnBytesLeaf layout");
struct DByteVecSeg {
  const void* tiles;
  const int32_t* vnorm2;
  const int32_t* ord_to_doc;
  int32_t doc_base, max_doc, n_vec, pad;
};
static_assert(sizeof(DByteVecSeg) == 40, "DByteVecSeg layout");

struct alignas(16) DKnnGatherLeaf {
  const void* rows;
  const int32_t* vnorm2;
  const int32_t* ord_to_doc;
  const uint64_t* accept;
  int64_t row_begin;
  int32_t n_rows, doc_base;
  int32_t max_doc, pad[3];
};
static_assert(sizeof(DKnnGatherLeaf) == 64, "DKnnGatherLeaf layout");

__host__ __device__ inline float knn_byte_score(int sim, int32_t dim, int32_t dot, int32_t nq, int32_t nv) {
  if (sim == 0) {
// ... 27 lines not shown
```

### nrtsearch_amd/csrc/planner.cpp

```cpp
#include "runtime_internal.h"



int nrtgpu::rt::validate_query(const nrtgpu_bm25_query& q, int qi) {
  if (q.k <= 0) return fail(NRTGPU_ERR_INVALID_ARG, "query %d: numHits must be > 0; got %d", qi, q.k);
  if (q.total_hits_threshold < 0) return fail(NRTGPU_ERR_INVALID_ARG, "query %d: totalHitsThreshold must be >= 0, got %d", qi, q.total_hits_threshold);
  if (q.k > NRTGPU_MAX_K) return fail(NRTGPU_ERR_UNSUPPORTED, "query %d: numHits %d > %d", qi, q.k, NRTGPU_MAX_K);
  if (q.n_terms <= 0 || !q.terms) return fail(NRTGPU_ERR_INVALID_ARG, "query %d: no terms", qi);
  if (q.n_terms > NRTGPU_MAX_TERMS) return fail(NRTGPU_ERR_UNSUPPORTED, "query %d: %d clauses > %d", qi, q.n_terms, NRTGPU_MAX_TERMS);
  if (q.min_should_match < 0) return fail(NRTGPU_ERR_INVALID_ARG, "query %d: minimumNumberShouldMatch %d", qi, q.min_should_match);
  if (q.disjunction_max != 0 && q.disjunction_max != 1) return fail(NRTGPU_ERR_INVALID_ARG, "query %d: disjunction_max must be 0 or 1", qi);
  if (q.disjunction_max == 1 && q.min_should_match > 1)
    return fail(NRTGPU_ERR_UNSUPPORTED, "query %d: a DisjunctionMaxQuery has no minimumNumberShouldMatch", qi);
  if (!(q.tie_breaker >= 0.0f && q.tie_breaker <= 1.0f)) return fail(NRTGPU_ERR_INVALID_ARG, "query %d: tie_breaker must be in [0, 1]", qi);
  if (q.tie_breaker != 0.0f && q.disjunction_max != 1) return fail(NRTGPU_ERR_INVALID_ARG, "query %d: tie_breaker without disjunction_max", qi);
  {
    int n_must = 0;
    for (int t = 0; t < q.n_terms; ++t) {
      if (q.terms[t].occur != 0 && q.terms[t].occur != 1) return fail(NRTGPU_ERR_INVALID_ARG, "query %d term %d: occur must be 0 (SHOULD) or 1 (MUST)", qi, t);
      n_must += q.terms[t].occur;
    }
    if (n_must != 0 && q.disjunction_max == 1) return fail(NRTGPU_ERR_INVALID_ARG, "query %d: the disjuncts of a DisjunctionMaxQuery have no occur", qi);
    if (n_must != 0 && q.min_should_match > 0)
      return fail(NRTGPU_ERR_UNSUPPORTED, "query %d: MUST clauses next to minimumNumberShouldMatch > 0", qi);
// ... 270 lines not shown
    bool fx_ok = true;
    int32_t fx_E = kNoFixed;
    for (int t = 0; t < q.n_terms && fx_ok; ++t) {
      if (term_total[(size_t)t] == 0) continue;
      const uint32_t max_norm = ents[(size_t)t]->max_norm;
      int32_t sc = 0;
      fx_ok = fixed_scale_of_term(q.terms[t].weight, q.norm_cache + (size_t)q.terms[t].cache_slot * 256, max_norm, &sc);
      term_scale[(size_t)t] = sc;
      if (fx_ok) fx_E = std::max(fx_E, sc);
    }
    for (int t = 0; t < q.n_terms && fx_ok; ++t)
      if (term_total[(size_t)t] != 0 && fx_E - term_scale[(size_t)t] > 15) fx_ok = false;
    if (!fx_ok) fx_E = kNoFixed;
    int64_t lower = 0;
    uint8_t route = kRouteScan;
    if (prune != 0 && fx_ok && q.n_terms <= kMsMaxTerms && !(q.min_competitive_score > 0.0f)) {
      const bool shaped = effective_msm(q) > 1 || q.filter_mask != 0 || q.must_not_mask != 0 || q.n_more_filters != 0 || q.n_more_must_not != 0 ||
                          sec_mode_of(q) == kMsSecReqOpt;
      if (q.total_hits_threshold == INT32_MAX) {
        int64_t all = 0;
        for (int t = 0; t < q.n_terms; ++t) all += term_total[(size_t)t];
        if (all > 0 && all <= kMsExactMaxPostings) route = kRouteMs + (uint8_t)kMsModeExact;
      } else {
        if (!shaped) {
          const int64_t floor_ = std::max<int64_t>(q.total_hits_threshold, q.k);
          int64_t best_slice = 0;
          for (int t = 0; t < q.n_terms; ++t) {
            const uint32_t* cnt = ents[(size_t)t]->count.data();
            int64_t certain = 0;
            if (n_slices <= 1) {
              certain = term_total[(size_t)t];
              if (any_deleted) {
                certain = 0;
                for (int si = 0; si < n_segs; ++si) certain += std::max<int64_t>(0, (int64_t)cnt[si] - n_deleted[si]);
              }
              best_slice = std::max(best_slice, certain);
            } else {
              std::fill(slice_sum.begin(), slice_sum.end(), 0);
              for (int si = 0; si < n_segs; ++si) {
                const int64_t c = std::max<int64_t>(0, (int64_t)cnt[si] - n_deleted[si]);
                slice_sum[(size_t)slice_of_leaf[si]] += c;
                certain += c;
              }
              for (int sl = 0; sl < n_slices; ++sl) best_slice = std::max(best_slice, slice_sum[(size_t)sl]);
            }
            lower = std::max(lower, certain);
          }
          if (best_slice <= floor_) lower = 0;
        }
        route = kRouteMs + (uint8_t)(lower > 0 ? kMsModePrune : kMsModeCount);
      }
    }
    q_lower[(size_t)qi] = lower;
    q_route[(size_t)qi] = route;
    {
      int64_t p0 = 0, p1 = 0;
      float w0 = -1.0f, w1 = -1.0f;
      for (int t = 0; t < q.n_terms; ++t) {
        if (term_total[(size_t)t] == 0) continue;
        const float wt = q.terms[t].weight;
        if (wt > w0) { w1 = w0; p1 = p0; w0 = wt; p0 = term_total[(size_t)t]; }
        else if (wt > w1) { w1 = wt; p1 = term_total[(size_t)t]; }
      }
      q_ms_key[(size_t)qi] = p0 + p1;
    }
    for (int t = 0; t < q.n_terms; ++t) tab_of_term[t] = -1;
    QTabs& qt_ = qtabs[(size_t)qi];
    qt_.n = 0;
    qt_.fx_E = fx_E;
    for (int r = 0; r < kTabTerms && r < q.n_terms; ++r) {
      int best = -1;
      for (int t = 0; t < q.n_terms; ++t)
        if (tab_of_term[(size_t)t] < 0 && term_total[(size_t)t] > 0 && (best < 0 || term_total[(size_t)t] > term_total[(size_t)best])) best = t;
      if (best < 0) break;
      tab_of_term[(size_t)best] = (int32_t)qt_.n;
      qt_.weight[qt_.n] = q.terms[best].weight;
      qt_.cache[qt_.n] = (uint32_t)q.terms[best].cache_slot;
      qt_.scale[qt_.n] = term_scale[(size_t)best];
      qt_.n++;
    }
    DQExpand& qx = qexpand[(size_t)qi];
    qx.term_begin = (uint32_t)pc.qterms.size();
    qx.by_weight = route != kRouteScan ? 1u : 0u;
    qx.pad = 0;
    const uint32_t* cnt_of[kMaxTerms];
    bool req_of[kMaxTerms];
    uint32_t n_live = 0;
    const bool req_opt = sec_mode_of(q) == kMsSecReqOpt;
    bool no_hits = false;
    for (int t = 0; t < q.n_terms; ++t) {
      const TermLeaves& tl = *ents[(size_t)t];
      if (tl.total <= 0) {
        no_hits = no_hits || (req_opt && q.terms[t].occur == 1);
        continue;
      }
      req_of[n_live] = req_opt && q.terms[t].occur == 1;
      DQTerm d{};
      d.table = tl.d_table;
      d.weight = q.terms[t].weight;
      d.cache_slot = (uint32_t)q.terms[t].cache_slot;
      d.tab_slot = (tab_of_term[(size_t)t] >= 0 ? (uint32_t)tab_of_term[(size_t)t] : kTabSlotNone) |
                   (sec_mode_of(q) == kMsSecReqOpt && q.terms[t].occur == 1 ? kTabSlotRequired : 0u);
      d.fx_scale = term_scale[(size_t)t];
      d.fx_shift = fx_ok ? (uint32_t)(fx_E - term_scale[(size_t)t]) : 0u;
      pc.qterms.push_back(d);
      cnt_of[n_live++] = tl.count.data();
    }
    qx.n_terms = n_live;
    q_qs_begin[qi] = (uint32_t)pc.qs.size();
    for (int si = 0; si < n_segs; ++si) {
      uint32_t n = 0;
      int64_t postings = 0;
      bool lacks_must = no_hits;
      for (uint32_t t = 0; t < n_live; ++t) {
        const uint32_t c = cnt_of[t][si];
        n += c != 0u ? 1u : 0u;
        postings += c;
        lacks_must = lacks_must || (req_of[t] && c == 0u);
      }
      if (lacks_must) n = 0;
      qs_begin[(size_t)qi * (size_t)n_segs + (size_t)si] = n ? pc.n_dterms : 0xFFFFFFFFu;
      if (n == 0) continue;
      pc.qs.push_back(QS{pc.n_dterms, n, si, postings});
      pc.n_dterms += n;
      pc.postings += postings;
      pc.cost += postings + (int64_t)segs[si]->n_tiles * kTileCostPostings;
    }
    q_qs_cnt[qi] = (uint32_t)pc.qs.size() - q_qs_begin[qi];
  }
}

int nrtgpu::rt::build_plan(nrtgpu_ctx* ctx, const nrtgpu_seg* const* segs, const int32_t* doc_bases, int32_t n_segs,
                      const nrtgpu_bm25_query* queries, int32_t n_queries, HostPlan& hp, int prune) {
  const double t_entry = now_ms();
  uint32_t kmax = 1;
  for (int qi = 0; qi < n_queries; ++qi) {
    if (int rc = validate_query(queries[qi], qi)) return rc;
    kmax = std::max<uint32_t>(kmax, (uint32_t)queries[qi].k);
  }
  for (int si = 0; si < n_segs; ++si) {
    if (!segs[si]) return fail(NRTGPU_ERR_INVALID_ARG, "segment %d is NULL", si);
    if (!segs[si]->sealed) return fail(NRTGPU_ERR_STATE, "segment %d is not sealed", si);
    if (segs[si]->ctx != ctx) return fail(NRTGPU_ERR_INVALID_ARG, "segment %d belongs to another context", si);
  }
  hp.k_stride = round_up(kmax, 16);
  hp.queries.resize((size_t)n_queries);
  hp.q_k.resize((size_t)n_queries);
  hp.theta_init.resize((size_t)n_queries);
  for (int qi = 0; qi < n_queries; ++qi)
    hp.theta_init[(size_t)qi] = queries[qi].min_competitive_score > 0.0f ? pack_key(queries[qi].min_competitive_score, 0xFFFFFFFFu) : 0ull;

  static const bool plan_trace = dev_env_int("NRTGPU_PLAN_TRACE", 0) != 0;
  const double tp0 = plan_trace ? now_ms() : 0.0;
  std::vector<uint32_t> q_qs_begin((size_t)n_queries), q_qs_cnt((size_t)n_queries);
  std::vector<uint32_t> cache_base((size_t)n_queries);
  std::vector<QTabs> qtabs((size_t)n_queries);
  int n_thr = ctx->cfg.host_threads > 0 ? ctx->cfg.host_threads : 4;
  n_thr = std::max(1, std::min(n_thr, n_queries / 64));
  static const long alone_below = dev_env_int("NRTGPU_PLAN_ALONE_PAIRS", 2048);
  if ((int64_t)n_queries * std::max(n_segs, 1) < alone_below) n_thr = 1;
  const int n_chunks = n_thr == 1 ? 1 : std::max(n_thr, std::min(n_queries / 64, 4 * n_thr));
  std::vector<PlanPiece> pieces((size_t)n_chunks);
  auto chunk_begin = [&](int t) { return (int)((int64_t)n_queries * t / n_chunks); };
  {
    const int variant = (ctx->cfg.flags >> 8) & 15;
    if ((ctx->cfg.flags & (NRTGPU_FLAG_NO_PRUNE | NRTGPU_FLAG_NO_FIXED_POINT)) != 0 || !(variant == 0 || variant == 7)) prune = 0;
  }
  hp.q_lower.assign((size_t)n_queries, 0);
  hp.q_route.assign((size_t)n_queries, kRouteScan);
  std::vector<int64_t> q_ms_key((size_t)n_queries, 0);
  hp.lsc = leaf_set_cache(ctx, segs, n_segs);
  hp.n_leaves = (uint32_t)n_segs;
  hp.qexpand.resize((size_t)n_queries);
  hp.qs_begin.assign((size_t)n_queries * (size_t)std::max(n_segs, 1), 0xFFFFFFFFu);
  std::vector<int32_t> n_deleted((size_t)std::max(n_segs, 1), 0);
  for (int si = 0; si < n_segs; ++si) n_deleted[(size_t)si] = segs[si]->n_deleted;
  std::vector<int32_t> slice_of_leaf((size_t)std::max(n_segs, 1), 0);
  int32_t n_slices = 1;
  if (n_segs > 0 && (int32_t)g_thread_slices.size() == n_segs) {
    std::unordered_map<int32_t, int32_t> dense;
    for (int32_t i = 0; i < n_segs; ++i) {
      auto it = dense.emplace(g_thread_slices[(size_t)i], (int32_t)dense.size()).first;
      slice_of_leaf[(size_t)i] = it->second;
    }
    n_slices = (int32_t)std::max<size_t>(dense.size(), 1);
  } else if (ctx->slice_max_docs.load() > 0 && n_segs > 0) {
    std::vector<hostmath::LeafInfo> all((size_t)n_segs);
    int32_t base = 0;
    for (int32_t i = 0; i < n_segs; ++i) {
      all[(size_t)i] = {i, segs[i]->max_doc, segs[i]->max_doc - segs[i]->n_deleted, doc_bases ? doc_bases[i] : base};
      base += segs[i]->max_doc;
    }
    const int32_t vs = ctx->virtual_shards.load();
    const std::vector<std::vector<int32_t>> sl = vs > 1
        ? hostmath::slices_for_shards(all, vs, ctx->slice_max_docs.load(), ctx->slice_max_segments.load(), nullptr)
        : hostmath::slices(all, ctx->slice_max_docs.load(), ctx->slice_max_segments.load(), all);
    n_slices = (int32_t)std::max<size_t>(sl.size(), 1);
    for (size_t s_ = 0; s_ < sl.size(); ++s_)
      for (int32_t li : sl[s_]) slice_of_leaf[(size_t)li] = (int32_t)s_;
  }
  auto work = [&](int t) {
    resolve_queries(*hp.lsc, segs, n_segs, n_deleted.data(), slice_of_leaf.data(), n_slices, queries, chunk_begin(t), chunk_begin(t + 1), pieces[(size_t)t],
                    q_qs_begin.data(), q_qs_cnt.data(), hp.qs_begin.data(), hp.qexpand.data(), cache_base, qtabs, prune, hp.q_lower, hp.q_route, q_ms_key);
  };
  ctx->pool->run(n_chunks, work);
  const double tp1 = plan_trace ? now_ms() : 0.0;
  int64_t total_postings = 0;
  {
    size_t nt = 0, nc = 0;
    for (const PlanPiece& pc : pieces) { nt += pc.qterms.size(); nc += pc.caches.size(); }
    hp.qterms.reserve(nt);
    hp.caches.reserve(nc);
  }
  std::vector<int> piece_of((size_t)n_queries, 0);
  for (int t = 0; t < n_chunks; ++t) {
    PlanPiece& pc = pieces[(size_t)t];
    if (pc.oom) return fail(NRTGPU_ERR_OOM, "out of device memory for the resident term tables");
    const uint32_t qterm_base = (uint32_t)hp.qterms.size(), c_base = (uint32_t)hp.caches.size(), dterm_base = hp.n_dterms;
    hp.qterms.insert(hp.qterms.end(), pc.qterms.begin(), pc.qterms.end());
    hp.caches.insert(hp.caches.end(), pc.caches.begin(), pc.caches.end());
    for (QS& qs : pc.qs) qs.term_begin += dterm_base;
    for (int qi = chunk_begin(t); qi < chunk_begin(t + 1); ++qi) {
      cache_base[(size_t)qi] += c_base;
      hp.qexpand[(size_t)qi].term_begin += qterm_base;
      piece_of[(size_t)qi] = t;
      if (dterm_base)
        for (int si = 0; si < n_segs; ++si) {
          uint32_t& b = hp.qs_begin[(size_t)qi * (size_t)n_segs + (size_t)si];
          if (b != 0xFFFFFFFFu) b += dterm_base;
        }
    }
    hp.n_dterms += pc.n_dterms;
    total_postings += pc.postings;
  }
  auto qs_of = [&](int qi) { return pieces[(size_t)piece_of[(size_t)qi]].qs.data() + q_qs_begin[(size_t)qi]; };
  hp.postings = total_postings;
  auto on_ms_kernel = [&](uint32_t q_) { return hp.q_route[q_] != kRouteScan; };
  hp.fixed_point = (ctx->cfg.flags & NRTGPU_FLAG_NO_FIXED_POINT) == 0;
  for (int qi = 0; qi < n_queries && hp.fixed_point; ++qi)
    if (!on_ms_kernel((uint32_t)qi) && q_qs_cnt[(size_t)qi] != 0 && qtabs[(size_t)qi].fx_E == kNoFixed) hp.fixed_point = false;
  for (int qi = 0; qi < n_queries; ++qi)
    if (on_ms_kernel((uint32_t)qi))
      for (uint32_t j = 0; j < q_qs_cnt[(size_t)qi]; ++j) hp.ms_postings += qs_of(qi)[j].postings;
  hp.clause_counting = false;
  hp.ms_shapes = false;
  hp.ms_two = false;
  for (int qi = 0; qi < n_queries; ++qi) {
    const nrtgpu_bm25_query& q = queries[qi];
    if (effective_msm(q) > 1 || q.disjunction_max == 1) (on_ms_kernel((uint32_t)qi) ? hp.ms_shapes : hp.clause_counting) = true;
    if (sec_mode_of(q) != kMsSecNone) {
      if (!on_ms_kernel((uint32_t)qi) && q_qs_cnt[(size_t)qi] != 0)
        return fail(NRTGPU_ERR_UNSUPPORTED, "query %d: a tie breaker > 0 / MUST next to SHOULD clauses run on the MaxScore route only (<= %d clauses, "
                                            "fixed-point sums, no min_competitive_score, not ScoreMode.COMPLETE over more than %lld postings)",
                    qi, kMsMaxTerms, (long long)kMsExactMaxPostings);
      hp.ms_two = true;
    }
    if ((q.filter_mask != 0 || q.must_not_mask != 0 || q.n_more_filters != 0 || q.n_more_must_not != 0) && on_ms_kernel((uint32_t)qi)) hp.ms_shapes = true;
  }
  hp.n_slices = (uint32_t)n_slices;
  if (hp.clause_counting && !hp.fixed_point)
    return fail(NRTGPU_ERR_UNSUPPORTED, "minimumNumberShouldMatch > 1 / DisjunctionMaxQuery need the fixed-point accumulators (weights of "
                                        "a query in this batch span too many binades, or NRTGPU_FLAG_NO_FIXED_POINT is set)");

  const double tp2 = plan_trace ? now_ms() : 0.0;
  const int64_t target_items = ctx->cfg.target_items > 0 ? ctx->cfg.target_items : (int64_t)std::max(ctx->n_cus, 1);
  const int64_t min_item_cost = 1 << 17;
  struct Pending { int64_t cost; uint32_t query; uint32_t part_begin, n_parts; uint32_t tiles; int32_t first_slice, last_slice; uint32_t n_slices; };
  std::vector<Pending> pend;
  std::vector<int64_t> q_costs((size_t)n_queries, 0), q_items((size_t)n_queries, 0);
  for (int qi = 0; qi < n_queries; ++qi)
    for (uint32_t j = 0; j < q_qs_cnt[(size_t)qi]; ++j) {
      const QS& qs = qs_of(qi)[j];
      q_costs[(size_t)qi] += qs.postings + (int64_t)segs[qs.seg]->n_tiles * kTileCostPostings;
    }
  hostmath::plan_item_counts(q_costs.data(), n_queries, target_items, min_item_cost, q_items.data());
  struct CutPiece { std::vector<DPart> parts; std::vector<Pending> pend; bool masked = false; int rc = 0; };
  std::vector<CutPiece> cuts((size_t)n_chunks);
  auto cut_work = [&](int t) {
    const int q0 = chunk_begin(t), q1 = chunk_begin(t + 1);
    std::vector<DPart>& parts = cuts[(size_t)t].parts;
    std::vector<Pending>& pend = cuts[(size_t)t].pend;
    bool& masked = cuts[(size_t)t].masked;
    int& cut_rc = cuts[(size_t)t].rc;
    std::vector<QS> by_slice;
    parts.reserve((size_t)(q1 - q0) * (size_t)std::max(n_segs, 1));
    pend.reserve((size_t)(q1 - q0) * 2);
    for (int qi = q0; qi < q1; ++qi) {
      const int64_t q_cost = q_costs[(size_t)qi];
      if (q_cost == 0) continue;
      const int64_t n_it = q_items[(size_t)qi];
      const double budget = (double)q_cost / (double)n_it;
      const QS* qsv = qs_of(qi);
      const uint32_t n_qs = q_qs_cnt[(size_t)qi];
      if (n_slices > 1) {
        by_slice.assign(qsv, qsv + n_qs);
        std::stable_sort(by_slice.begin(), by_slice.end(), [&](const QS& a, const QS& b) { return slice_of_leaf[(size_t)a.seg] < slice_of_leaf[(size_t)b.seg]; });
        qsv = by_slice.data();
      }
      const bool scan_route = hp.q_route[(size_t)qi] == kRouteScan;
      Pending cur{0, (uint32_t)qi, (uint32_t)parts.size(), 0, 0, -1, -1, 0};
      double filled = 0.0;
      auto close_item = [&]() {
        pend.push_back(cur);
        cur = Pending{0, (uint32_t)qi, (uint32_t)parts.size(), 0, 0, -1, -1, 0};
        filled = 0.0;
      };
// ... 176 lines not shown
```

### nrtsearch_amd/csrc/runtime_internal.h

```cpp
#pragma once
#include <hip/hip_runtime.h>
#include <fcntl.h>
#include <stdarg.h>
#include <stdio.h>
#include <string.h>
#include <sys/mman.h>
#include <unistd.h>

#include <algorithm>
#include <atomic>
#include <cerrno>
#include <climits>
#include <cmath>
#include <chrono>
#include <condition_variable>
#include <deque>
#include <functional>
#include <map>
#include <memory>
#include <mutex>
#include <optional>
#include <shared_mutex>
#include <string>
#include <thread>
#include <unordered_map>
#include <vector>

#include "../../include/nrtgpu.h"
#ifdef NRTGPU_DEV
#include "../../include/nrtgpu_dev.h"
#endif
#include "host_math.h"
#include "plan.h"

namespace nrtgpu {
void launch_bm25_scan(hipStream_t stream, bool fixed_point, bool pipelined, bool packed, int ablation, uint32_t n_items, const DItem* items,
                      const DPart* parts, const DTerm* terms, const DQuery* queries, const float* caches, unsigned long long* theta_g,
                      unsigned long long* quant_g, const DExchange* xch, uint32_t* slice_sum, uint64_t* item_keys, uint32_t* item_counts,
                      uint64_t* item_hits, uint32_t k_stride, uint64_t* item_prof);
void launch_bm25_maxscore(hipStream_t stream, bool profile, bool packed, int shapes, const MsArgs& args, const MsArgs* args_d);
#ifdef NRTGPU_DEV
void launch_debug_wave_kth(hipStream_t stream, const uint64_t* keys, uint32_t n, uint32_t r, uint64_t* out);
#endif
void launch_term_frontier(hipStream_t stream, const uint32_t* fnorm, const uint64_t* t_start, const uint32_t* t_count,
                          const uint64_t* t_look, const uint32_t* t_meta, const void* look_base, uint32_t n_terms, DTermAux* out);
void launch_term_bits(hipStream_t stream, const uint32_t* docids, const uint64_t* t_start, const uint32_t* t_count, const uint64_t* t_look,
                      const uint32_t* which, uint32_t n_which, uint32_t max_count, void* look_base);
void launch_term_cells(hipStream_t stream, const uint32_t* docids, const uint64_t* t_start, const uint32_t* t_count, const uint64_t* t_look,
                       const uint32_t* t_meta, const uint32_t* which, uint32_t n_which, uint32_t max_cells, uint32_t max_doc, void* look_base);
void launch_expand_terms(hipStream_t stream, const DQExpand* qx, const DQTerm* qterms, const uint32_t* out_begin, uint32_t n_queries,
                         uint32_t n_leaves, DTerm* out);
void launch_slice_relation(hipStream_t stream, const uint32_t* slice_sum, const DQuery* queries, uint32_t n_slices, uint64_t* out_hits,
                           uint32_t n);
void launch_patch_hits(hipStream_t stream, const uint64_t* lower, uint64_t* hits, uint32_t n);
void launch_merge_topk(hipStream_t stream, uint32_t n_queries, const uint64_t* in_keys, const uint32_t* in_counts,
                       const uint64_t* in_hits, const uint32_t* list_idx, const uint32_t* q_base,
                       const uint32_t* q_nlists, uint32_t k_stride_in, const uint32_t* q_k, uint64_t* out_keys,
                       uint32_t* out_counts, uint64_t* out_hits, uint32_t k_stride_out, const uint32_t* help_query = nullptr,
                       uint32_t n_help = 0, uint32_t help_slot_base = 0, const unsigned long long* spec_g = nullptr);
void launch_fold_norms(hipStream_t stream, const uint32_t* docids, const uint32_t* freqs, const uint8_t* norms,
                       uint32_t* fnorm, uint64_t n, uint32_t* overflow);
void launch_pack_count(hipStream_t stream, const uint32_t* fnorm, uint64_t n, uint32_t n_blocks, uint32_t* counts);
void launch_pack_write(hipStream_t stream, const uint32_t* docids, const uint32_t* fnorm, uint64_t n, uint32_t n_blocks,
                       const uint32_t* dir, uint32_t* exceptions, uint32_t* packed);
void launch_apply_live(hipStream_t stream, const uint32_t* docids, uint32_t* fnorm, uint64_t n, const uint64_t* live);
void launch_knn_row_norms(hipStream_t st, const float* vecs, int32_t dim, int64_t n, float* norm2);
int launch_knn_score(hipStream_t st, uint32_t blocks, const float* vecs, const float* vnorm2, const int32_t* ord_to_doc,
                     const uint64_t* live_bits, int32_t dim, int64_t row_begin, int64_t row_end, int32_t doc_base,
                     const float* qpanel, const float* qnorm2, int32_t n_q, int32_t sim, float boost,
                     const unsigned long long* theta, uint64_t* cand, uint32_t* cand_cnt, uint32_t cap, int32_t append_only = 0);
void launch_knn_select(hipStream_t st, uint32_t n_q, uint64_t* topk, uint32_t* topk_cnt, uint32_t k_stride, uint32_t k,
                       const uint64_t* cand, uint32_t* cand_cnt, uint32_t cap, unsigned long long* theta,
                       uint32_t* overflow);
void launch_knn_refine_select(hipStream_t st, uint32_t n_q, uint64_t* topk, uint32_t* topk_cnt, uint32_t k_stride, uint32_t k,
                              const uint64_t* cand, uint32_t* cand_cnt, uint32_t cap, unsigned long long* theta, uint32_t* overflow,
                              const DVecSeg* segs, int32_t n_segs, int32_t dim, int32_t sim, const float* qpanel, const float* qnorm2,
                              float boost, const float* ebound, float erel, float min_score, uint32_t k_int, int32_t certify,
                              uint32_t* cert);
void launch_knn_norm_max(hipStream_t st, const float* norm2, int64_t n, uint32_t* out_bits);
void launch_knn_norm_min(hipStream_t st, const float* norm2, int64_t n, uint32_t* out_bits);
void launch_knn_absmax(hipStream_t st, const float* vecs, int64_t n_elems, uint32_t* out_bits);
size_t knn_sketch_bytes(int32_t dim, int64_t n);
size_t knn_sketch_lds_bytes(int32_t dim, int32_t n_q);
bool knn_sketch_fits(int32_t dim, int32_t n_q);
void launch_knn_panel_fp16(hipStream_t st, const float* qpanel, const float* qscale, int32_t dim, int32_t n_q, void* panel16);
void launch_knn_sketch_build(hipStream_t st, const float* vecs, int32_t dim, int64_t n, float scale, void* sketch);
int launch_knn_sketch(hipStream_t st, uint32_t blocks, const DKnnLeaf* leaves, int32_t n_leaves, int32_t dim, int64_t tile_begin,
                      int64_t tile_end, const void* panel16, const float* qnorm2, const float* qscale, int32_t n_q, int32_t sim,
                      float boost, const unsigned long long* theta, uint64_t* cand, uint32_t* cand_cnt, uint32_t cap, int32_t append_only = 0);
void launch_rescore_vectors(hipStream_t st, const float* vecs, const float* vnorm2, int32_t dim, const float* query,
                            float qnorm2, int32_t sim, float boost, const int64_t* vec_row, const float* first_scores,
                            int32_t n, double qw, double rw, float* out_scores);
void launch_hybrid_rescore(hipStream_t st, uint32_t n_queries, const uint64_t* first_keys, const uint32_t* first_counts,
                           uint32_t k_stride, const DVecSeg* segs, int32_t n_segs, int32_t dim, const float* qvecs,
                           const float* qnorm2, int32_t sim, float boost, double qw, double rw, uint32_t window,
                           uint64_t* out_keys, uint32_t* out_counts, uint32_t w_stride, int32_t drop_foreign = 0);
void launch_hybrid_hits(hipStream_t st, const uint64_t* first_hits, const uint32_t* first_counts, const uint32_t* q_k, int32_t carries,
                        uint64_t* out_hits, uint32_t n);
int32_t knn_bytes_steps(int32_t dim);
size_t knn_bytes_tile_bytes(int32_t dim, int64_t n);
size_t knn_bytes_panel_bytes(int32_t dim, int32_t n_q);
void launch_knn_bytes_pack(hipStream_t st, const int8_t* rows, int32_t dim, int64_t row0, int64_t n_chunk, void* tiles, int32_t* norm2);
int launch_knn_bytes(hipStream_t st, uint32_t blocks, const DKnnBytesLeaf* leaves, int32_t n_leaves, int32_t dim, int64_t tile_begin,
                     int64_t tile_end, const void* panel, const int32_t* qnorm2, int32_t n_q, int32_t sim, float boost, float min_score,
                     const unsigned long long* theta, uint64_t* cand, uint32_t* cand_cnt, uint32_t cap, int32_t append_only = 0);
void launch_rescore_byte_vectors(hipStream_t st, const void* tiles, const int32_t* vnorm2, int32_t dim, const void* query, int32_t qnorm2,
                                 int32_t sim, float boost, const int64_t* vec_row, const float* first_scores, int32_t n, double qw, double rw,
                                 float* out_scores);
void launch_hybrid_rescore_bytes(hipStream_t st, uint32_t n_queries, const uint64_t* first_keys, const uint32_t* first_counts,
                                 uint32_t k_stride, const DByteVecSeg* segs, int32_t n_segs, int32_t dim, const void* qvecs,
                                 const int32_t* qnorm2, int32_t sim, float boost, double qw, double rw, uint32_t window, uint64_t* out_keys,
                                 uint32_t* out_counts, uint32_t w_stride);
int launch_knn_accept_rows(hipStream_t st, const DKnnGatherLeaf* leaves, int32_t n_leaves, int64_t total_rows, uint64_t* list, uint32_t* count,
                           uint32_t cap);
int launch_knn_gather_score(hipStream_t st, const DKnnGatherLeaf* leaves, const uint64_t* list, const uint32_t* count, uint32_t max_rows,
                            int32_t dim, const float* qpanel, const float* qnorm2, int32_t n_q, int32_t sim, float boost, float min_score,
                            uint64_t* cand, uint32_t* cand_cnt, uint32_t cap);
int launch_knn_gather_bytes(hipStream_t st, const DKnnGatherLeaf* leaves, const uint64_t* list, const uint32_t* count, uint32_t max_rows,
                            int32_t dim, const void* queries, const int32_t* qnorm2, int32_t n_q, int32_t sim, float boost, float min_score,
                            uint64_t* cand, uint32_t* cand_cnt, uint32_t cap);
}

namespace nrtgpu {
namespace rt {

// ... 603 lines not shown
```

### nrtsearch_amd/csrc/search.cpp

```cpp
#include "runtime_internal.h"


static uint32_t spec_margin16(const nrtgpu_ctx* ctx) { return (uint32_t)std::max(ctx->spec_z16.load(std::memory_order_relaxed), 0); }
static void spec_sync_epoch(const nrtgpu_ctx* ctx, LeafSetCache* lsc) {
  const uint64_t e = ctx->spec_epoch.load(std::memory_order_relaxed);
  if (lsc->spec_epoch.exchange(e, std::memory_order_relaxed) != e) {
    lsc->spec_queries.store(0, std::memory_order_relaxed);
    lsc->spec_reruns.store(0, std::memory_order_relaxed);
    lsc->spec_calls.store(0, std::memory_order_relaxed);
    lsc->spec_calls_rerun.store(0, std::memory_order_relaxed);
    lsc->spec_scattered.store(0, std::memory_order_relaxed);
    lsc->spec_off.store(0, std::memory_order_relaxed);
  }
}
static bool speculating(nrtgpu_ctx* ctx, const nrtgpu_seg* const* segs, int32_t n_segs) {
  if (!ctx || spec_margin16(ctx) == 0u || !segs || n_segs <= 0) return false;
  for (int32_t i = 0; i < n_segs; ++i)
    if (!segs[i]) return false;
  std::shared_ptr<LeafSetCache> lsc = leaf_set_cache(ctx, segs, n_segs);
  spec_sync_epoch(ctx, lsc.get());
  return lsc->spec_off.load(std::memory_order_relaxed) == 0;
}
static void note_speculation_of(nrtgpu_ctx* ctx, LeafSetCache* lsc, int64_t n_queries, int64_t n_rerun) {
  spec_sync_epoch(ctx, lsc);
  const int64_t seen = lsc->spec_queries.fetch_add(n_queries, std::memory_order_relaxed) + n_queries;
  const int64_t failed = lsc->spec_reruns.fetch_add(n_rerun, std::memory_order_relaxed) + n_rerun;
  ctx->spec_queries.fetch_add(n_queries, std::memory_order_relaxed);
  ctx->spec_reruns.fetch_add(n_rerun, std::memory_order_relaxed);
  const int64_t calls = lsc->spec_calls.fetch_add(1, std::memory_order_relaxed) + 1;
  const int64_t calls_bad = lsc->spec_calls_rerun.fetch_add(n_rerun > 0 ? 1 : 0, std::memory_order_relaxed) + (n_rerun > 0 ? 1 : 0);
  const bool no_verdict = dev_env_int("NRTGPU_SPEC_NO_VERDICT", 0) != 0;
  if (((seen >= 2048 && failed * 50 > seen) || (calls >= 32 && calls_bad * 4 > calls)) && !no_verdict) {
    if (lsc->spec_scattered.exchange(1, std::memory_order_relaxed) == 0) {
      lsc->spec_queries.store(0, std::memory_order_relaxed);
      lsc->spec_reruns.store(0, std::memory_order_relaxed);
      lsc->spec_calls.store(0, std::memory_order_relaxed);
      lsc->spec_calls_rerun.store(0, std::memory_order_relaxed);
      ctx->spec_scattered.store(1, std::memory_order_relaxed);
    } else {
      lsc->spec_off.store(1, std::memory_order_relaxed);
      ctx->spec_off.store(1, std::memory_order_relaxed);
    }
  }
}
static void note_speculation(nrtgpu_ctx* ctx, const nrtgpu_seg* const* segs, int32_t n_segs, int64_t n_queries, int64_t n_rerun) {
  std::shared_ptr<LeafSetCache> lsc = leaf_set_cache(ctx, segs, n_segs);
  note_speculation_of(ctx, lsc.get(), n_queries, n_rerun);
}

void nrtgpu::rt::note_shard_speculation(nrtgpu_ctx* ctx, const nrtgpu_seg* const* segs, int32_t n_segs, int64_t n_queries, int64_t n_failed) {
  note_speculation(ctx, segs, n_segs, n_queries, n_failed);
}

static bool ms_persistent() {
  static const bool v = dev_env_int("NRTGPU_MS_PERSISTENT", 1) != 0;
  return v;
}

struct DeviceRun {
  uint64_t* out_keys = nullptr;
  uint32_t* out_counts = nullptr;
  uint64_t* out_hits = nullptr;
  uint64_t* prof = nullptr;
  size_t n_items = 0;
  size_t n_slots = 0;
  uint64_t* walls = nullptr;
  size_t n_ms_items = 0;
};

static int enqueue_search(nrtgpu_ctx* ctx, Slot* slot, const HostPlan& hp, int32_t n_queries, uint32_t k_stride_out,
                          uint64_t* ext_keys, uint32_t* ext_counts, uint64_t* ext_hits, DeviceRun* run,
                          std::unique_lock<std::mutex>& gpu, int64_t epoch = -1, bool allow_spec = false, int32_t spec_world = 1,
                          uint64_t* ext_guess = nullptr, bool follow_up = false) {
  forget_foreign_hip_error();
  static const bool follow_up_on = dev_env_int("NRTGPU_FOLLOW_UP", 1) != 0;
  const bool small = follow_up && follow_up_on && hp.n_ms_items != 0 && hp.n_ms_items == hp.items.size() && ms_persistent();
  const size_t n_items = hp.items.size();
  Carver pc;
  const size_t o_queries = pc.take(hp.queries.size() * sizeof(DQuery));
  const size_t o_items = pc.take(n_items * sizeof(DItem));
  const size_t o_parts = pc.take(hp.parts.size() * sizeof(DPart));
  const size_t o_qterms = pc.take(hp.qterms.size() * sizeof(DQTerm));
  const size_t o_qexp = pc.take(hp.qexpand.size() * sizeof(DQExpand));
  const size_t o_qsb = pc.take(hp.qs_begin.size() * 4);
  const size_t o_caches = pc.take(hp.caches.size() * sizeof(float));
  const size_t o_lidx = pc.take(hp.list_idx.size() * 4);
  const size_t o_qbase = pc.take(hp.q_base.size() * 4);
  const size_t o_qnl = pc.take(hp.q_nlists.size() * 4);
  const size_t o_qk = pc.take(hp.q_k.size() * 4);
  const size_t o_theta = pc.take(hp.theta_init.size() * 8);
  const size_t o_quant = pc.take(hp.list_idx.size() * 8);
  const size_t o_lower = pc.take(ext_hits ? hp.q_lower.size() * 8 : 0);
  const bool use_xch = epoch >= 0 && ctx->xch_dev != nullptr;
  const size_t o_xch = pc.take(use_xch ? sizeof(DExchange) : 0);
  const size_t o_qwins = pc.take(hp.q_wins.size() * 4);
  const size_t o_help = pc.take(sizeof(MsArgs));
  const size_t plan_bytes = pc.off;
  if (int rc = slot->h_plan.reserve(plan_bytes)) return rc;
  if (int rc = slot->d_plan.reserve(plan_bytes)) return rc;
  char* hb = (char*)slot->h_plan.p;
  memcpy(hb + o_queries, hp.queries.data(), hp.queries.size() * sizeof(DQuery));
  if (n_items) memcpy(hb + o_items, hp.items.data(), n_items * sizeof(DItem));
  if (!hp.parts.empty()) memcpy(hb + o_parts, hp.parts.data(), hp.parts.size() * sizeof(DPart));
  if (!hp.qterms.empty()) memcpy(hb + o_qterms, hp.qterms.data(), hp.qterms.size() * sizeof(DQTerm));
  memcpy(hb + o_qexp, hp.qexpand.data(), hp.qexpand.size() * sizeof(DQExpand));
  if (!hp.qs_begin.empty()) memcpy(hb + o_qsb, hp.qs_begin.data(), hp.qs_begin.size() * 4);
  memcpy(hb + o_caches, hp.caches.data(), hp.caches.size() * sizeof(float));
  if (!hp.list_idx.empty()) memcpy(hb + o_lidx, hp.list_idx.data(), hp.list_idx.size() * 4);
  memcpy(hb + o_qbase, hp.q_base.data(), hp.q_base.size() * 4);
  memcpy(hb + o_qnl, hp.q_nlists.data(), hp.q_nlists.size() * 4);
  memcpy(hb + o_qk, hp.q_k.data(), hp.q_k.size() * 4);
  memcpy(hb + o_theta, hp.theta_init.data(), hp.theta_init.size() * 8);
  if (!hp.q_wins.empty()) memcpy(hb + o_qwins, hp.q_wins.data(), hp.q_wins.size() * 4);
  if (spec_world > 1) {
    uint64_t num = (uint64_t)spec_world, den = 1;
    const int64_t sd = ctx->shard_docs.load(std::memory_order_relaxed), id = ctx->index_docs.load(std::memory_order_relaxed);
    if (sd > 0 && id >= sd) {
      num = (uint64_t)id;
      den = (uint64_t)sd;
    }
    uint32_t* qw = (uint32_t*)(hb + o_qwins);
    for (size_t i = 0; i < hp.q_wins.size(); ++i) qw[i] = (uint32_t)std::min<uint64_t>(((uint64_t)qw[i] * num + den - 1) / den, 0xFFFFFFFFull);
  }
  memset(hb + o_quant, 0, hp.list_idx.size() * 8);
  if (ext_hits) memcpy(hb + o_lower, hp.q_lower.data(), hp.q_lower.size() * 8);
  if (use_xch) {
    DExchange x{};
    const size_t stride = (size_t)ctx->cfg.max_batch;
    x.slot = ctx->xch_dev + (size_t)(epoch % kExchangeSlots) * (size_t)ctx->xch_world * stride;
    x.world = (uint32_t)ctx->xch_world;
    x.rank = (uint32_t)ctx->xch_rank;
    x.stride = (uint32_t)stride;
    x.tag = (uint32_t)(epoch + 1);
    if (x.tag == 0) x.tag = 1;
    memcpy(hb + o_xch, &x, sizeof(x));
  }

  static const int env_helpers = (int)dev_env_int("NRTGPU_MS_HELPERS", -1);
  static const int env_help_min = (int)dev_env_int("NRTGPU_MS_HELP_MIN", 16);
  const size_t n_help = hp.n_ms_items == 0 ? 0 : (size_t)(env_helpers >= 0 ? env_helpers : 4 * std::max(ctx->n_cus, 1));
  const size_t n_slots = n_items + n_help;
  Carver wc;
  const size_t o_ikeys = wc.take(n_slots * (size_t)hp.k_stride * 8);
  const size_t o_icnt = wc.take(n_slots * 4);
  const size_t o_ihits = wc.take(n_slots * 8);
  const size_t o_okeys = wc.take((size_t)n_queries * k_stride_out * 8);
  const size_t o_ocnt = wc.take((size_t)n_queries * 4);
  const size_t o_ohits = wc.take((size_t)n_queries * 8);
  const size_t o_terms = wc.take((size_t)hp.n_dterms * sizeof(DTerm));
  const size_t o_ssum = wc.take((size_t)n_queries * hp.n_slices * 4), o_qprune = wc.take((size_t)n_queries * 4);
  const size_t o_hwin = wc.take(hp.n_ms_items * 4), o_hcnt = wc.take(hp.n_ms_items * 4), o_ht0 = wc.take(hp.n_ms_items * 8);
  const size_t o_hhead = wc.take((size_t)n_queries * 4), o_hnext = wc.take(n_help * 4), o_hoff = wc.take(4);
  const size_t o_hqueue = wc.take(4), o_hused = wc.take(4), o_hstart = wc.take(8);
  const uint32_t spec_z16 = spec_margin16(ctx);
  const bool spec = allow_spec && spec_z16 != 0u && hp.n_ms_items != 0 && !use_xch && hp.lsc && hp.lsc->spec_off.load(std::memory_order_relaxed) == 0;
  const size_t o_spec = wc.take(spec ? (size_t)n_queries * 8 : 0);
  const size_t zero_bytes = wc.off - o_ssum;
  const int flag_variant = (ctx->cfg.flags >> 8) & 15;
  const int ablation = hp.clause_counting ? 8 : ((hp.masked && flag_variant == 0 && !(ctx->cfg.flags & NRTGPU_FLAG_NO_MASK_VARIANT)) ? 9 : flag_variant);
  const bool profile = flag_variant == 7;
  const size_t o_prof = wc.take((ablation == 7 || profile) ? n_slots * 128 : 0);
  const size_t o_walls = wc.take(profile ? n_slots * 64 : 0);
  if (int rc = slot->d_work.reserve(wc.off)) return rc;
  char* db = (char*)slot->d_plan.p;
  char* wb = (char*)slot->d_work.p;
  DHelp help{};
  help.win_next = (uint32_t*)(wb + o_hwin);
  help.help_cnt = (uint32_t*)(wb + o_hcnt);
  help.item_t0 = (unsigned long long*)(wb + o_ht0);
  help.help_head = (uint32_t*)(wb + o_hhead);
  help.help_query = (uint32_t*)(wb + o_hnext);
  help.help_off = (uint32_t*)(wb + o_hoff);
  help.item_next = (uint32_t*)(wb + o_hqueue);
  help.help_used = (uint32_t*)(wb + o_hused);
  help.t_start = (unsigned long long*)(wb + o_hstart);
  {
    static const int env_help_alpha = (int)dev_env_int("NRTGPU_MS_HELP_ALPHA", 24);
    uint64_t wins = 0;
    for (size_t i = 0; i < hp.n_ms_items; ++i) wins += hp.items[i].flags >> 8;
    help.total_wins = (uint32_t)std::min<uint64_t>(wins, 0xFFFFFFFFull);
    help.alpha16 = (uint32_t)std::max(env_help_alpha, 0);
    static const int env_spare = (int)dev_env_int("NRTGPU_MS_SPARE_CUS", 8);
    help.n_cus = (uint32_t)std::max(ctx->n_cus - std::max(env_spare, 0), 1);
    if (small) help.n_cus = (uint32_t)std::max(env_spare, 1);
    help.persistent = ms_persistent() ? 1u : 0u;
  }
  help.n_own = (uint32_t)hp.n_ms_items;
  help.n_help = (uint32_t)n_help;
  help.slot_base = (uint32_t)n_items;
  static const bool env_help_greedy = dev_env_int("NRTGPU_MS_HELP_GREEDY", 0) != 0;
  help.min_rem = (uint32_t)std::min(std::max(env_help_min, 1), 0xFFFF) | (env_help_greedy ? 1u << 16 : 0u);
  help.walls = profile ? (unsigned long long*)(wb + o_walls) : nullptr;
  help.spec_g = spec ? (unsigned long long*)(wb + o_spec) : nullptr;
  help.spec_z16 = spec ? spec_z16 : 0u;
  {
    const int env_first = (int)dev_env_int("NRTGPU_MS_SPEC_FIRST", 2 * kMsWaves);
    const int env_grow = (int)dev_env_int("NRTGPU_MS_SPEC_GROW", 32);
    const bool env_meet = dev_env_int("NRTGPU_MS_SPEC_MEET", 0) != 0;
    help.spec_sched = (uint32_t)std::min(std::max(env_first, 1), 255) | ((uint32_t)std::min(std::max(env_grow, 17), 255) << 8) | (env_meet ? 1u << 16 : 0u);
  }
  MsArgs ms_args{};
  ms_args.items = (const DItem*)(db + o_items);
  ms_args.parts = (const DPart*)(db + o_parts);
  ms_args.terms = (const DTerm*)(wb + o_terms);
  ms_args.queries = (const DQuery*)(db + o_queries);
  ms_args.caches = (const float*)(db + o_caches);
  ms_args.theta_g = (unsigned long long*)(db + o_theta);
  ms_args.slice_sum = (uint32_t*)(wb + o_ssum);
  ms_args.q_prune = (uint32_t*)(wb + o_qprune);
  ms_args.xch = use_xch ? (const DExchange*)(db + o_xch) : nullptr;
  ms_args.item_keys = (uint64_t*)(wb + o_ikeys);
  ms_args.item_counts = (uint32_t*)(wb + o_icnt);
  ms_args.item_hits = (uint64_t*)(wb + o_ihits);
  ms_args.item_prof = profile ? (uint64_t*)(wb + o_prof) : nullptr;
  ms_args.q_wins = (const uint32_t*)(db + o_qwins);
  {
    const long forced = dev_env_int("NRTGPU_MS_SCATTER", -1);
    ms_args.scatter = forced >= 0 ? (forced != 0 ? 1u : 0u) : ((spec && hp.lsc->spec_scattered.load(std::memory_order_relaxed) != 0) ? 1u : 0u);
  }
  ms_args.k_stride = hp.k_stride;
  ms_args.help = help;
  memcpy(hb + o_help, &ms_args, sizeof(ms_args));

  hipStream_t st = slot->stream;
  HIP_TRY(hipMemcpyAsync(db, hb, plan_bytes, hipMemcpyHostToDevice, st));
  HIP_TRY(hipMemsetAsync(wb + o_ssum, 0, zero_bytes, st));
  const bool timing = ctx->cfg.collect_timing != 0;
  const size_t n_ms = hp.n_ms_items;
  launch_expand_terms(st, (const DQExpand*)(db + o_qexp), (const DQTerm*)(db + o_qterms), (const uint32_t*)(db + o_qsb),
                      (uint32_t)n_queries, hp.n_leaves, (DTerm*)(wb + o_terms));
  gpu.lock();
  static const bool overlap_scorers = dev_env_int("NRTGPU_OVERLAP_SCORERS", 0) != 0;
  if (ctx->last_turn && !overlap_scorers && !small) HIP_TRY(hipStreamWaitEvent(st, ctx->last_turn, 0));
  if (ctx->last_knn_turn) HIP_TRY(hipStreamWaitEvent(st, ctx->last_knn_turn, 0));
  if (timing) HIP_TRY(hipEventRecord(slot->ev3, st));
  if (profile && n_help) HIP_TRY(hipMemsetAsync(wb + o_prof + n_items * 128, 0, n_help * 128, st));
  if (profile) HIP_TRY(hipMemsetAsync(wb + o_walls, 0, n_slots * 64, st));
  launch_bm25_maxscore(st, profile, (ctx->cfg.flags & NRTGPU_FLAG_PACKED_POSTINGS) != 0, hp.ms_two ? 2 : (hp.ms_shapes ? 1 : 0), ms_args, (const MsArgs*)(db + o_help));
  if (timing) HIP_TRY(hipEventRecord(slot->ev0, st));
  launch_bm25_scan(st, hp.fixed_point, (ctx->cfg.flags & NRTGPU_FLAG_NO_PREFETCH) == 0, (ctx->cfg.flags & NRTGPU_FLAG_PACKED_POSTINGS) != 0, ablation, (uint32_t)(n_items - n_ms),
                   (const DItem*)(db + o_items) + n_ms, (const DPart*)(db + o_parts), (const DTerm*)(wb + o_terms),
                   (const DQuery*)(db + o_queries), (const float*)(db + o_caches),
                   (unsigned long long*)(db + o_theta), (unsigned long long*)(db + o_quant),
                   use_xch ? (const DExchange*)(db + o_xch) : nullptr, (uint32_t*)(wb + o_ssum), (uint64_t*)(wb + o_ikeys) + n_ms * (size_t)hp.k_stride,
                   (uint32_t*)(wb + o_icnt) + n_ms, (uint64_t*)(wb + o_ihits) + n_ms, hp.k_stride,
                   ablation == 7 ? (uint64_t*)(wb + o_prof) + n_ms * 16 : nullptr);
  if (timing) HIP_TRY(hipEventRecord(slot->ev1, st));
  static const bool turn_before_merge = dev_env_int("NRTGPU_TURN_BEFORE_MERGE", 1) != 0;
  if (turn_before_merge && !small) {
    HIP_TRY(hipEventRecord(slot->ev_turn, st));
    ctx->last_turn = slot->ev_turn;
  }
  uint64_t* okeys = ext_keys ? ext_keys : (uint64_t*)(wb + o_okeys);
  uint32_t* ocnt = ext_counts ? ext_counts : (uint32_t*)(wb + o_ocnt);
  uint64_t* ohits = ext_hits ? ext_hits : (uint64_t*)(wb + o_ohits);
  launch_merge_topk(st, (uint32_t)n_queries, (const uint64_t*)(wb + o_ikeys), (const uint32_t*)(wb + o_icnt),
                    (const uint64_t*)(wb + o_ihits), (const uint32_t*)(db + o_lidx), (const uint32_t*)(db + o_qbase),
                    (const uint32_t*)(db + o_qnl), hp.k_stride, (const uint32_t*)(db + o_qk), okeys, ocnt, ohits,
                    k_stride_out, n_help ? help.help_query : nullptr, (uint32_t)n_help, help.slot_base, spec_world > 1 ? nullptr : help.spec_g);
  if (ext_guess) {
    if (spec) HIP_TRY(hipMemcpyAsync(ext_guess, wb + o_spec, (size_t)n_queries * 8, hipMemcpyDeviceToDevice, st));
    else HIP_TRY(hipMemsetAsync(ext_guess, 0, (size_t)n_queries * 8, st));
  }
  launch_slice_relation(st, (const uint32_t*)(wb + o_ssum), (const DQuery*)(db + o_queries), hp.n_slices, ohits, (uint32_t)n_queries);
  if (ext_hits && hp.n_ms_items) launch_patch_hits(st, (const uint64_t*)(db + o_lower), ohits, (uint32_t)n_queries);
  if (timing) HIP_TRY(hipEventRecord(slot->ev2, st));
  if (!turn_before_merge && !small) {
    HIP_TRY(hipEventRecord(slot->ev_turn, st));
    ctx->last_turn = slot->ev_turn;
  }
  gpu.unlock();
  HIP_TRY(hipGetLastError());
  run->out_keys = okeys;
  run->out_counts = ocnt;
  run->out_hits = ohits;
  run->prof = (ablation == 7 || profile) ? (uint64_t*)(wb + o_prof) : nullptr;
  run->n_items = n_items;
  run->n_slots = n_slots;
  run->walls = profile ? (uint64_t*)(wb + o_walls) : nullptr;
  run->n_ms_items = n_ms;
  return 0;
}

static void account(nrtgpu_ctx* ctx, Slot* slot, const HostPlan& hp, int32_t n_queries, double plan_ms, double t_entry_ms = 0.0,
                    double queue_ms = 0.0) {
  float scan_ms = 0.f, merge_ms = 0.f, ms_ms = 0.f;
  if (ctx->cfg.collect_timing) {
    (void)hipEventElapsedTime(&ms_ms, slot->ev3, slot->ev0);
    (void)hipEventElapsedTime(&scan_ms, slot->ev0, slot->ev1);
    (void)hipEventElapsedTime(&merge_ms, slot->ev1, slot->ev2);
  }
  const size_t n_scan = hp.items.size() - hp.n_ms_items;
  {
    nrtgpu_diagnostics d{};
    d.total_ms = t_entry_ms > 0.0 ? now_ms() - t_entry_ms : 0.0;
    d.plan_ms = plan_ms;
    d.queue_ms = queue_ms;
    d.device_ms = (double)(hp.n_ms_items ? ms_ms : 0.f) + (double)(n_scan ? scan_ms : 0.f) + (double)merge_ms;
// ... 903 lines not shown
```

Baseline: 522,600.

## Precompute per-term walk rows in expand kernel and find parts with a wave scan

Moves per-clause setup (upper bound, suffix sums, flags, look/cell pointers) out of the maxscore kernel and into the expand_terms kernel. Expand now writes an 80-byte DWalkRow per term that the maxscore wave copies into LDS with vector loads. Part lookup for items with at most 64 parts is replaced by a lane-parallel prefix scan plus a ballot, instead of a serial loop. This cuts redundant per-window setup work and latency in the hot kernel, in exchange for extra work and memory in the expand kernel and a new workspace buffer. Debug entry points are added to check the rows.

```diff
diff --git a/include/nrtgpu_dev.h b/include/nrtgpu_dev.h
--- a/include/nrtgpu_dev.h
+++ b/include/nrtgpu_dev.h
@@ -21,6 +21,11 @@
 int  nrtgpu_get_maxscore_profile(nrtgpu_ctx* ctx, double* out16);
 int  nrtgpu_debug_maxscore_meetings(nrtgpu_ctx* ctx, int64_t* out4);
 int  nrtgpu_debug_wave_kth(const uint64_t* keys, int32_t n, int32_t r, uint64_t* out);
+int64_t nrtgpu_debug_walk_rows(nrtgpu_ctx* ctx, const nrtgpu_seg* const* segs, const int32_t* doc_bases, int32_t n_segs,
+                               const nrtgpu_bm25_query* queries, int32_t n_queries, int32_t* out_begin, int32_t* out_n,
+                               uint64_t* out_rows, int64_t cap_rows);
+int  nrtgpu_debug_walk_value(float weight, const uint32_t* freq, const uint32_t* norm, int32_t n, const float* table256, int32_t fx_scale,
+                             uint32_t fx_shift, uint64_t* out);
 int64_t nrtgpu_get_maxscore_item_walls(nrtgpu_ctx* ctx, uint64_t* out, int64_t cap_slots, int64_t* n_items);
 
 #ifdef __cplusplus
diff --git a/nrtsearch_amd/_lib.py b/nrtsearch_amd/_lib.py
--- a/nrtsearch_amd/_lib.py
+++ b/nrtsearch_amd/_lib.py
@@ -49,7 +49,7 @@
     "nrtgpu_bench_closed_loop", "nrtgpu_debug_hold_coalescers", "nrtgpu_debug_coalescer_pending", "nrtgpu_debug_live_segments",
     "nrtgpu_debug_spec_counters", "nrtgpu_get_scan_profile", "nrtgpu_get_maxscore_profile", "nrtgpu_get_maxscore_item_walls",
     "nrtgpu_debug_dist_inject", "nrtgpu_debug_term_lookup", "nrtgpu_debug_knn_bounds",
-    "nrtgpu_debug_maxscore_meetings", "nrtgpu_debug_wave_kth",
+    "nrtgpu_debug_maxscore_meetings", "nrtgpu_debug_wave_kth", "nrtgpu_debug_walk_rows", "nrtgpu_debug_walk_value",
 ]
 DEV_LIB_PATH = os.path.join(_HERE, "libnrtgpu_dev.so")
 
@@ -209,6 +209,10 @@
     if hasattr(L, "nrtgpu_debug_maxscore_meetings"):
         L.nrtgpu_debug_maxscore_meetings.argtypes = [vp, vp]
         L.nrtgpu_debug_wave_kth.argtypes = [vp, i32, i32, vp]
+    if hasattr(L, "nrtgpu_debug_walk_rows"):
+        L.nrtgpu_debug_walk_rows.argtypes = [vp, vp, vp, i32, vp, i32, vp, vp, vp, i64]
+        L.nrtgpu_debug_walk_rows.restype = C.c_int64
+        L.nrtgpu_debug_walk_value.argtypes = [f32, vp, vp, i32, vp, i32, C.c_uint32, vp]
     if hasattr(L, "nrtgpu_debug_knn_bounds"):
         L.nrtgpu_debug_knn_bounds.argtypes = [i32, i32, C.c_double, C.c_double, f32, C.c_double, C.c_double, f32, f32, C.c_double, C.c_double, vp]
     L.nrtgpu_set_slicing.argtypes = [vp, i32, i32, i32]
diff --git a/nrtsearch_amd/api.py b/nrtsearch_amd/api.py
--- a/nrtsearch_amd/api.py
+++ b/nrtsearch_amd/api.py
@@ -547,6 +547,22 @@
     def search(self, query: Query, manager: TopScoreDocCollectorManager) -> TopDocs:
         return self.search_batch([query], [manager])[0]
 
+    def debug_walk_rows(self, queries: Sequence[Query], managers: Sequence[TopScoreDocCollectorManager]):
+        n, nl = len(queries), len(self.leaves)
+        m = self._marshal(queries, managers)
+        begin = np.full((n, nl), -1, dtype=np.int32)
+        count = np.zeros((n, nl), dtype=np.int32)
+        L = _lib.load()
+        total = int(L.nrtgpu_debug_walk_rows(self.ctx._h, self._segs, self._bases, nl, m.queries, n, begin.ctypes.data, count.ctypes.data, None, 0))
+        if total < 0:
+            _lib.check(-total)
+        rows = np.zeros(max(total, 1), dtype=WALK_ROW_DTYPE)
+        got = int(L.nrtgpu_debug_walk_rows(self.ctx._h, self._segs, self._bases, nl, m.queries, n, begin.ctypes.data, count.ctypes.data,
+                                           rows.ctypes.data, total))
+        if got < 0:
+            _lib.check(-got)
+        return begin, count, rows[:total]
+
     def dist_search_batch(self, queries: Sequence[Query], managers: Sequence[TopScoreDocCollectorManager],
                           mode: int = EXCHANGE_ALLGATHER) -> List[Optional[TopDocs]]:
         n = len(queries)
@@ -911,6 +927,22 @@
     return int(out[0])
 
 
+WALK_ROW_DTYPE = np.dtype([("docids", "<u8"), ("fnorm", "<u8"), ("suffix", "<u8"), ("ub", "<u8"), ("weight", "<f4"), ("fx_scale", "<i4"),
+                           ("flags", "<u4"), ("pad", "<u4"), ("u_after", "<u8"), ("look", "<u8"), ("cells", "<u8"), ("start", "<u8")])
+assert WALK_ROW_DTYPE.itemsize == 80
+
+
+def debug_walk_value(weight: float, freqs, norm_bytes, table256: np.ndarray, fx_scale: int, fx_shift: int) -> np.ndarray:
+    f = np.ascontiguousarray(freqs, dtype=np.uint32)
+    nb = np.ascontiguousarray(norm_bytes, dtype=np.uint32)
+    tab = np.ascontiguousarray(table256, dtype=np.float32)
+    assert f.shape == nb.shape and f.ndim == 1 and tab.shape == (256,)
+    out = np.zeros(len(f), dtype=np.uint64)
+    _lib.check(_lib.load().nrtgpu_debug_walk_value(C.c_float(float(weight)), f.ctypes.data, nb.ctypes.data, len(f), tab.ctypes.data, int(fx_scale),
+                                                  int(fx_shift), out.ctypes.data))
+    return out
+
+
 def blend(retriever_docs: Sequence[np.ndarray], retriever_scores: Optional[Sequence[np.ndarray]] = None,
           boosts: Optional[Sequence[float]] = None, mode: str = "rrf", k: int = 60, start_hit: int = 0, top_hits: int = 10) -> TopDocs:
     n = len(retriever_docs)
diff --git a/nrtsearch_amd/csrc/devtools.cpp b/nrtsearch_amd/csrc/devtools.cpp
--- a/nrtsearch_amd/csrc/devtools.cpp
+++ b/nrtsearch_amd/csrc/devtools.cpp
@@ -93,3 +93,81 @@
   if (e != hipSuccess) return fail(NRTGPU_ERR_HIP, "wave_kth: %s", hipGetErrorString(e));
   return NRTGPU_OK;
 }
+
+extern "C" int64_t nrtgpu_debug_walk_rows(nrtgpu_ctx* ctx, const nrtgpu_seg* const* segs, const int32_t* doc_bases, int32_t n_segs,
+                                          const nrtgpu_bm25_query* queries, int32_t n_queries, int32_t* out_begin, int32_t* out_n,
+                                          uint64_t* out_rows, int64_t cap_rows) {
+  if (!ctx || !segs || !queries || !out_begin || !out_n || (!out_rows && cap_rows > 0)) return -(int64_t)fail(NRTGPU_ERR_INVALID_ARG, "NULL argument");
+  if (n_queries <= 0 || n_segs <= 0 || cap_rows < 0) return -(int64_t)fail(NRTGPU_ERR_INVALID_ARG, "n_queries and n_segs must be > 0");
+  if (hipSetDevice(ctx->device) != hipSuccess) return -(int64_t)fail(NRTGPU_ERR_HIP, "hipSetDevice");
+  for (int si = 0; si < n_segs; ++si)
+    if (!segs[si]) return -(int64_t)fail(NRTGPU_ERR_INVALID_ARG, "segment %d is NULL", si);
+  SegReadLocks content(segs, n_segs);
+  HostPlan hp;
+  if (int rc = build_plan(ctx, segs, doc_bases, n_segs, queries, n_queries, hp, 1)) return -(int64_t)rc;
+  const size_t n_pairs = (size_t)n_queries * (size_t)n_segs;
+  for (size_t i = 0; i < n_pairs; ++i) out_begin[i] = -1, out_n[i] = 0;
+  if (hp.n_dterms == 0) return 0;
+  Carver c;
+  const size_t o_qx = c.take(sizeof(DExpandHead) + hp.qexpand.size() * sizeof(DQExpand)) + sizeof(DExpandHead), o_qt = c.take(hp.qterms.size() * sizeof(DQTerm));
+  const size_t o_qsb = c.take(hp.qs_begin.size() * 4), o_caches = c.take(hp.caches.size() * sizeof(float));
+  const size_t o_queries = c.take(hp.queries.size() * sizeof(DQuery)), o_up = c.off;
+  const size_t o_terms = c.take((size_t)hp.n_dterms * sizeof(DTerm)), o_rows = c.take((size_t)hp.n_dterms * sizeof(DWalkRow));
+  std::vector<char> hb(c.off, 0);
+  memcpy(hb.data() + o_qx, hp.qexpand.data(), hp.qexpand.size() * sizeof(DQExpand));
+  if (!hp.qterms.empty()) memcpy(hb.data() + o_qt, hp.qterms.data(), hp.qterms.size() * sizeof(DQTerm));
+  memcpy(hb.data() + o_qsb, hp.qs_begin.data(), hp.qs_begin.size() * 4);
+  if (!hp.caches.empty()) memcpy(hb.data() + o_caches, hp.caches.data(), hp.caches.size() * sizeof(float));
+  memcpy(hb.data() + o_queries, hp.queries.data(), hp.queries.size() * sizeof(DQuery));
+  char* db = nullptr;
+  if (hipMalloc((void**)&db, c.off) != hipSuccess) return -(int64_t)fail(NRTGPU_ERR_OOM, "hipMalloc");
+  DExpandHead xh{};
+  xh.caches = (const float*)(db + o_caches);
+  xh.queries = (const DQuery*)(db + o_queries);
+  xh.rows = (DWalkRow*)(db + o_rows);
+  memcpy(hb.data() + o_qx - sizeof(DExpandHead), &xh, sizeof(xh));
+  hipError_t e = hipMemcpy(db, hb.data(), o_up, hipMemcpyHostToDevice);
+  if (e == hipSuccess) e = hipMemset(db + o_up, 0, c.off - o_up);
+  if (e == hipSuccess) {
+    launch_expand_terms(nullptr, (const DQExpand*)(db + o_qx), (const DQTerm*)(db + o_qt), (const uint32_t*)(db + o_qsb), (uint32_t)n_queries,
+                        hp.n_leaves, (DTerm*)(db + o_terms));
+    e = hipGetLastError();
+  }
+  if (e == hipSuccess) e = hipMemcpy(hb.data() + o_rows, db + o_rows, (size_t)hp.n_dterms * sizeof(DWalkRow), hipMemcpyDeviceToHost);
+  (void)hipFree(db);
+  if (e != hipSuccess) return -(int64_t)fail(NRTGPU_ERR_HIP, "walk_rows: %s", hipGetErrorString(e));
+  static_assert(sizeof(DWalkRow) == 80, "ten words per row");
+  if (out_rows) memcpy(out_rows, hb.data() + o_rows, (size_t)std::min<int64_t>(cap_rows, (int64_t)hp.n_dterms) * sizeof(DWalkRow));
+  std::vector<uint32_t> begins;
+  for (size_t i = 0; i < n_pairs; ++i)
+    if (hp.qs_begin[i] != 0xFFFFFFFFu) begins.push_back(hp.qs_begin[i]);
+  std::sort(begins.begin(), begins.end());
+  for (size_t i = 0; i < n_pairs; ++i) {
+    const uint32_t b = hp.qs_begin[i];
+    if (b == 0xFFFFFFFFu || hp.qexpand[i / (size_t)n_segs].by_weight == 0u) continue;
+    auto nx = std::upper_bound(begins.begin(), begins.end(), b);
+    out_begin[i] = (int32_t)b;
+    out_n[i] = (int32_t)((nx == begins.end() ? hp.n_dterms : *nx) - b);
+  }
+  return (int64_t)hp.n_dterms;
+}
+
+extern "C" int nrtgpu_debug_walk_value(float weight, const uint32_t* freq, const uint32_t* norm, int32_t n, const float* table256, int32_t fx_scale,
+                                       uint32_t fx_shift, uint64_t* out) {
+  if (!freq || !norm || !table256 || !out || n < 1 || fx_shift > 31u) return fail(NRTGPU_ERR_INVALID_ARG, "bad walk_value arguments");
+  char* d = nullptr;
+  const size_t o_f = 0, o_n = (size_t)n * 4, o_t = 2 * (size_t)n * 4, o_o = o_t + 1024, bytes = o_o + (size_t)n * 8;
+  if (hipMalloc((void**)&d, bytes) != hipSuccess) return fail(NRTGPU_ERR_OOM, "hipMalloc");
+  hipError_t e = hipMemcpy(d + o_f, freq, (size_t)n * 4, hipMemcpyHostToDevice);
+  if (e == hipSuccess) e = hipMemcpy(d + o_n, norm, (size_t)n * 4, hipMemcpyHostToDevice);
+  if (e == hipSuccess) e = hipMemcpy(d + o_t, table256, 1024, hipMemcpyHostToDevice);
+  if (e == hipSuccess) {
+    launch_debug_walk_value(nullptr, weight, (const uint32_t*)(d + o_f), (const uint32_t*)(d + o_n), (const float*)(d + o_t), fx_scale, fx_shift, (uint32_t)n,
+                            (uint64_t*)(d + o_o));
+    e = hipGetLastError();
+  }
+  if (e == hipSuccess) e = hipMemcpy(out, d + o_o, (size_t)n * 8, hipMemcpyDeviceToHost);
+  (void)hipFree(d);
+  if (e != hipSuccess) return fail(NRTGPU_ERR_HIP, "walk_value: %s", hipGetErrorString(e));
+  return NRTGPU_OK;
+}
diff --git a/nrtsearch_amd/csrc/kernels.hip b/nrtsearch_amd/csrc/kernels.hip
--- a/nrtsearch_amd/csrc/kernels.hip
+++ b/nrtsearch_amd/csrc/kernels.hip
@@ -954,6 +954,7 @@
   const uint32_t q = i / n_leaves, leaf = i - q * n_leaves;
   const DQExpand x = qx[q];
   const DQTerm* const qt = qterms + x.term_begin;
+  uint32_t n_here = 0;
   for (uint32_t t = 0; t < x.n_terms; ++t) {
     DTerm d = qt[t].table[leaf];
     if (d.docids == nullptr) continue;
@@ -976,6 +977,47 @@
     d.fx_scale = qt[t].fx_scale;
     d.fx_shift = qt[t].fx_shift;
     out[ob + rank] = d;
+    n_here += 1u;
+  }
+  if (x.by_weight == 0u) return;
+  const DExpandHead head = *((const DExpandHead*)qx - 1);
+  DWalkRow* const rows = head.rows;
+  if (rows == nullptr) return;
+  const float* const caches = head.caches;
+  const bool use_max = head.queries[q].combine_max != 0u;
+  uint64_t run = 0;
+  for (uint32_t c = n_here; c-- > 0u;) {
+    const DTerm d = out[ob + c];
+    const u32x4 a0 = ((const u32x4*)d.aux)[0], a1 = ((const u32x4*)d.aux)[1];
+    static_assert(offsetof(DTermAux, min_norm) == 8 && offsetof(DTermAux, esc_min_norm) == 20 && offsetof(DTermAux, esc_max_freq) == 24, "DTermAux layout");
+    const uint32_t mn[3] = {a0[2], a0[3], a1[0]};
+    const uint32_t esc_min_norm = a1[1] & 255u, look_kind = (a1[1] >> 8) & 255u, look_shift = (a1[1] >> 16) & 255u, esc_max_freq = a1[2];
+    const uint64_t look = ((uint64_t)a0[1] << 32) | a0[0];
+    const float* const cache = caches + x.cache_off + d.cache_slot * 256u;
+    uint32_t v = 0;
+#pragma unroll
+    for (uint32_t f = 0; f < 12u; ++f) {
+      const uint32_t nb = (mn[f >> 2] >> (8u * (f & 3u))) & 255u;
+      if (nb != 0xFFu) v = max(v, score_value<true>(bm25_score(d.weight, (float)(int32_t)(f + 1u), cache[nb]), d.fx_scale));
+    }
+    if (esc_max_freq != 0u)
+      v = max(v, score_value<true>(bm25_score(d.weight, (float)(int32_t)esc_max_freq, cache[esc_min_norm]), d.fx_scale));
+    const uint64_t ub = (uint64_t)v << d.fx_shift;
+    DWalkRow r;
+    r.docids = (uint64_t)d.docids;
+    r.fnorm = (uint64_t)d.fnorm;
+    r.ub = ub;
+    r.weight = d.weight;
+    r.fx_scale = d.fx_scale;
+    r.flags = walk_row_flags(d.tab_slot, d.fx_shift, d.cache_slot, d.shift, look_kind, look_shift, (d.tab_slot & kTabSlotRequired) != 0u);
+    r.pad = 0;
+    r.u_after = run;
+    run = use_max ? max(run, ub) : run + ub;
+    r.suffix = run;
+    r.look = look_kind != kLookNone ? look : 0ull;
+    r.cells = (uint64_t)d.cell_off;
+    r.start = d.start;
+    rows[ob + c] = r;
   }
 }
 void launch_expand_terms(hipStream_t stream, const DQExpand* qx, const DQTerm* qterms, const uint32_t* out_begin, uint32_t n_queries,
@@ -985,6 +1027,21 @@
   hipLaunchKernelGGL(expand_terms_kernel, dim3((uint32_t)((n + 255) / 256)), dim3(256), 0, stream, qx, qterms, out_begin, n_queries,
                      n_leaves, out);
 }
+
+#ifdef NRTGPU_DEV
+__global__ __launch_bounds__(256)
+void debug_walk_value_kernel(float weight, const uint32_t* __restrict__ freq, const uint32_t* __restrict__ norm, const float* __restrict__ table,
+                             int fx_scale, uint32_t fx_shift, uint32_t n, uint64_t* __restrict__ out) {
+  const uint32_t i = blockIdx.x * blockDim.x + threadIdx.x;
+  if (i >= n) return;
+  out[i] = (uint64_t)score_value<true>(bm25_score(weight, (float)(int32_t)freq[i], table[norm[i] & 255u]), fx_scale) << fx_shift;
+}
+void launch_debug_walk_value(hipStream_t stream, float weight, const uint32_t* freq, const uint32_t* norm, const float* table, int fx_scale,
+                             uint32_t fx_shift, uint32_t n, uint64_t* out) {
+  if (n == 0) return;
+  hipLaunchKernelGGL(debug_walk_value_kernel, dim3((n + 255u) / 256u), dim3(256), 0, stream, weight, freq, norm, table, fx_scale, fx_shift, n, out);
+}
+#endif
 
 __global__ __launch_bounds__(256)
 void slice_relation_kernel(const uint32_t* __restrict__ slice_sum, const DQuery* __restrict__ queries, uint32_t n_slices,
diff --git a/nrtsearch_amd/csrc/maxscore.hip b/nrtsearch_amd/csrc/maxscore.hip
--- a/nrtsearch_amd/csrc/maxscore.hip
+++ b/nrtsearch_amd/csrc/maxscore.hip
@@ -250,7 +250,10 @@
     const __attribute__((address_space(4))) DHelp& hp = ap->help;
     const DItem* const items = as_global(ap->items);
     const DPart* const parts = as_global(ap->parts);
+    const DWalkRow* const rows = as_global(ap->rows);
+  #ifdef NRTGPU_DEV
     const DTerm* const terms = as_global(ap->terms);
+  #endif
     const DExchange* const xch = as_global(ap->xch);
     bool helper = false;
     uint32_t my_item = 0, out_slot = 0;
@@ -449,19 +452,39 @@
     uint32_t pi = 0;
     uint32_t win_base = 0;
 
+    const bool parts_by_lane = item.n_parts <= 64u;
+    uint32_t part_incl = 0;
+    if (parts_by_lane) {
+      uint32_t w = 0;
+      if (lane < item.n_parts) {
+        const u32x2 tr = *(gvec2_ptr)&parts[item.part_begin + lane].tile_begin;
+        w = (tr[1] - (tr[0] & ~(win_tiles - 1u)) + win_tiles - 1u) / win_tiles;
+      }
+      part_incl = scan64_dpp(w);
+    }
+
     for (;;) {
       DPart part;
       uint32_t part_wins = 0;
-      if (sc_mul != 1u) {
-        pi = 0;
-        win_base = 0;
-      }
-      for (;; ++pi) {
-        if (pi >= item.n_parts) break;
+      if (parts_by_lane) {
+        const uint64_t holds = __builtin_amdgcn_ballot_w64(lane < item.n_parts && g < part_incl);
+        if (holds == 0ull) break;
+        pi = (uint32_t)__builtin_ctzll(holds);
         part = parts[item.part_begin + pi];
         part_wins = (part.tile_end - (part.tile_begin & ~(win_tiles - 1u)) + win_tiles - 1u) / win_tiles;
-        if (g < win_base + part_wins) break;
-        win_base += part_wins;
+        win_base = (uint32_t)__builtin_amdgcn_readlane((int)part_incl, (int)pi) - part_wins;
+      } else {
+        if (sc_mul != 1u) {
+          pi = 0;
+          win_base = 0;
+        }
+        for (;; ++pi) {
+          if (pi >= item.n_parts) break;
+          part = parts[item.part_begin + pi];
+          part_wins = (part.tile_end - (part.tile_begin & ~(win_tiles - 1u)) + win_tiles - 1u) / win_tiles;
+          if (g < win_base + part_wins) break;
+          win_base += part_wins;
+        }
       }
       if (pi >= item.n_parts) break;
       {
@@ -474,69 +497,92 @@
         if (lane == 0) s.slot_slice[p_slot] = part.slice & 0xFFFFFFu;
       }
       const uint32_t n_terms = part.n_terms;
-      const DTerm* const part_terms = terms + part.term_begin;
-
-      uint64_t my_ub = 0, my_suf = 0;
+      uint64_t my_suf = 0, my_start = 0;
+      gu32_ptr my_cells = nullptr;
+      uint32_t my_shift = 0, my_flags = 0;
       const uint64_t t_part0 = PROF ? __builtin_readcyclecounter() : 0ull;
-      const DTerm mt = part_terms[min(lane, n_terms - 1u)];
+  #ifdef NRTGPU_DEV
+      if (rows == nullptr) {
+        const DTerm* const part_terms = terms + part.term_begin;
+        uint64_t my_ub = 0;
+        const DTerm mt = part_terms[min(lane, n_terms - 1u)];
+        {
+          uint32_t ub_raw = 0;
+          for (uint32_t pass = 0; pass * 4u < n_terms; ++pass) {
+            const uint32_t tt = pass * 4u + (lane >> 4), i = lane & 15u;
+            const DTerm* Tp = part_terms + min(tt, n_terms - 1u);
+            const DTermAux* ax = Tp->aux;
+            const float w = Tp->weight;
+            const int scale = Tp->fx_scale;
+            const float* cache = &s.cache[Tp->cache_slot][0];
+            uint32_t v = 0;
+            if (tt < n_terms) {
+              if (i < 12u) {
+                const uint32_t nb = ax->min_norm[i];
+                if (nb != 0xFFu) v = score_value<true>(bm25_score(w, (float)(int32_t)(i + 1u), cache[nb]), scale);
+              } else if (i == 12u) {
+                const uint32_t mf = ax->esc_max_freq;
+                if (mf != 0u) v = score_value<true>(bm25_score(w, (float)(int32_t)mf, cache[ax->esc_min_norm]), scale);
+              }
+            }
+    #pragma unroll
+            for (int dlt = 8; dlt > 0; dlt >>= 1) v = max(v, (uint32_t)__shfl_xor((int)v, dlt, 64));
+            const uint32_t got = (uint32_t)__shfl((int)v, (int)((lane & 3u) * 16u), 64);
+            if ((lane >> 2) == pass) ub_raw = got;
+          }
+          if (lane < n_terms) my_ub = (uint64_t)ub_raw << mt.fx_shift;
+        }
+        uint64_t my_after = 0;
+        {
+          uint64_t run = 0;
+          for (int m = (int)n_terms - 1; m >= 0; --m) {
+            const uint64_t ub = readlane_u64(my_ub, (uint32_t)m);
+            if (lane == (uint32_t)m) my_after = run;
+            run = use_max ? max(run, ub) : run + ub;
+            if (lane == (uint32_t)m) my_suf = run;
+          }
+        }
+        my_cells = (gu32_ptr)mt.cell_off;
+        my_shift = mt.shift;
+        my_start = mt.start;
+        if (lane < n_terms) {
+          WClause w;
+          w.docids = (uint64_t)mt.docids;
+          w.fnorm = (uint64_t)mt.fnorm;
+          w.begin = 0;
+          w.count = w.pad0 = 0;
+          w.weight = mt.weight;
+          w.fx_scale = mt.fx_scale;
+          const DTermAux* const ax = mt.aux;
+          const uint32_t look_kind = ax->look_kind;
+          w.flags = ((mt.tab_slot & 0xFFFFu) < (uint32_t)kTabTerms ? (mt.tab_slot & 0xFFFFu) : 7u) | (TWO && (mt.tab_slot & kTabSlotRequired) ? 8u : 0u) |
+                    (mt.fx_shift << 4) | (mt.cache_slot << 8) | ((mt.shift & 31u) << 16) | ((look_kind & 7u) << 24) | (((uint32_t)ax->look_shift & 31u) << 27);
+          w.pad = 0;
+          w.u_after = my_after;
+          w.look = look_kind != kLookNone ? (uint64_t)ax->look : 0ull;
+          w.cells = (uint64_t)mt.cell_off;
+          w.start = mt.start;
+          wcl[lane] = w;
+          my_flags = w.flags;
+        }
+      } else
+  #endif
       {
-        uint32_t ub_raw = 0;
-        for (uint32_t pass = 0; pass * 4u < n_terms; ++pass) {
-          const uint32_t tt = pass * 4u + (lane >> 4), i = lane & 15u;
-          const DTerm* Tp = part_terms + min(tt, n_terms - 1u);
-          const DTermAux* ax = Tp->aux;
-          const float w = Tp->weight;
-          const int scale = Tp->fx_scale;
-          const float* cache = &s.cache[Tp->cache_slot][0];
-          uint32_t v = 0;
-          if (tt < n_terms) {
-            if (i < 12u) {
-              const uint32_t nb = ax->min_norm[i];
-              if (nb != 0xFFu) v = score_value<true>(bm25_score(w, (float)(int32_t)(i + 1u), cache[nb]), scale);
-            } else if (i == 12u) {
-              const uint32_t mf = ax->esc_max_freq;
-              if (mf != 0u) v = score_value<true>(bm25_score(w, (float)(int32_t)mf, cache[ax->esc_min_norm]), scale);
-            }
-          }
-  #pragma unroll
-          for (int dlt = 8; dlt > 0; dlt >>= 1) v = max(v, (uint32_t)__shfl_xor((int)v, dlt, 64));
-          const uint32_t got = (uint32_t)__shfl((int)v, (int)((lane & 3u) * 16u), 64);
-          if ((lane >> 2) == pass) ub_raw = got;
-        }
-        if (lane < n_terms) my_ub = (uint64_t)ub_raw << mt.fx_shift;
-      }
-      uint64_t my_after = 0;
-      {
-        uint64_t run = 0;
-        for (int m = (int)n_terms - 1; m >= 0; --m) {
-          const uint64_t ub = readlane_u64(my_ub, (uint32_t)m);
-          if (lane == (uint32_t)m) my_after = run;
-          run = use_max ? max(run, ub) : run + ub;
-          if (lane == (uint32_t)m) my_suf = run;
-        }
-      }
-      const gu32_ptr my_cells = (gu32_ptr)mt.cell_off;
-      const uint32_t my_shift = mt.shift;
-      if (lane < n_terms) {
-        WClause w;
-        w.docids = (uint64_t)mt.docids;
-        w.fnorm = (uint64_t)mt.fnorm;
-        w.begin = 0;
-        w.count = w.pad0 = 0;
-        w.weight = mt.weight;
-        w.fx_scale = mt.fx_scale;
-        const DTermAux* const ax = mt.aux;
-        const uint32_t look_kind = ax->look_kind;
-        w.flags = ((mt.tab_slot & 0xFFFFu) < (uint32_t)kTabTerms ? (mt.tab_slot & 0xFFFFu) : 7u) | (TWO && (mt.tab_slot & kTabSlotRequired) ? 8u : 0u) |
-                  (mt.fx_shift << 4) | (mt.cache_slot << 8) | ((mt.shift & 31u) << 16) | ((look_kind & 7u) << 24) | (((uint32_t)ax->look_shift & 31u) << 27);
-        w.pad = 0;
-        w.u_after = my_after;
-        w.look = look_kind != kLookNone ? (uint64_t)ax->look : 0ull;
-        w.cells = (uint64_t)mt.cell_off;
-        w.start = mt.start;
-        wcl[lane] = w;
-      }
-      const uint32_t req_mask = TWO ? (uint32_t)__builtin_amdgcn_ballot_w64(lane < n_terms && (mt.tab_slot & kTabSlotRequired) != 0u) : 0u;
+        static_assert(sizeof(DWalkRow) == sizeof(WClause) && sizeof(WClause) % 16 == 0, "a walk row is the image of a WClause");
+        const gvec_ptr src = (gvec_ptr)(rows + part.term_begin);
+        if (lane < n_terms * (uint32_t)(sizeof(WClause) / 16)) *(u32x4*)lds_ptr(wcl_addr + lane * 16u) = src[lane];
+        wave_lds_phase();
+        if (lane < n_terms) {
+          const uint32_t rec = wcl_addr + lane * (uint32_t)sizeof(WClause);
+          my_suf = *(const uint64_t*)lds_ptr(rec + 16u);
+          my_flags = *(const uint32_t*)lds_ptr(rec + 40u);
+          const u32x4 cs = *(const u32x4*)lds_ptr(rec + 64u);
+          my_cells = (gu32_ptr)(((uint64_t)cs[1] << 32) | cs[0]);
+          my_start = ((uint64_t)cs[3] << 32) | cs[2];
+        }
+        my_shift = (my_flags >> 16) & 31u;
+      }
+      const uint32_t req_mask = TWO ? (uint32_t)__builtin_amdgcn_ballot_w64(lane < n_terms && (my_flags & 8u) != 0u) : 0u;
       const uint32_t first_req = req_mask != 0u ? (uint32_t)__builtin_ctz(req_mask) : 0xFFu;
       if (PROF) tc_part += __builtin_readcyclecounter() - t_part0;
 
@@ -581,7 +627,7 @@
         uint32_t ng = 0;
         {
           const uint64_t thr_w = __hip_atomic_load(&s.prune_on, __ATOMIC_RELAXED, __HIP_MEMORY_SCOPE_WORKGROUP) ? loosen(max(s.thr, thr_other)) : 0ull;
-          const uint64_t pb = mt.start + my_lo, pe = mt.start + my_hi;
+          const uint64_t pb = my_start + my_lo, pe = my_start + my_hi;
           if (lane < n_terms) {
             if (my_suf >= thr_w && pe > pb && (!SHAPES || msm <= 1u || lane + msm <= n_terms) && (!TWO || lane <= first_req)) ng = (uint32_t)((pe - (pb & ~3ull) + (uint64_t)(kSl - 1)) / (uint64_t)kSl);
             *(u32x4*)&wcl[lane].begin = u32x4{(uint32_t)pb, (uint32_t)(pb >> 32), (uint32_t)(pe - pb), 0u};
diff --git a/nrtsearch_amd/csrc/plan.h b/nrtsearch_amd/csrc/plan.h
--- a/nrtsearch_amd/csrc/plan.h
+++ b/nrtsearch_amd/csrc/plan.h
@@ -65,9 +65,18 @@
   uint32_t term_begin;
   uint32_t n_terms;
   uint32_t by_weight;
-  uint32_t pad;
+  uint32_t cache_off;
 };
 static_assert(sizeof(DQExpand) == 16, "DQExpand layout");
+struct DWalkRow;
+struct DQuery;
+struct alignas(16) DExpandHead {
+  const float* caches;
+  const DQuery* queries;
+  DWalkRow* rows;
+  uint64_t pad;
+};
+static_assert(sizeof(DExpandHead) == 2 * sizeof(DQExpand), "the head takes the place of two DQExpand records");
 
 constexpr uint32_t kLookNone = 0, kLookBits = 1, kLookCells = 2;
 struct alignas(16) DTermAux {
@@ -81,6 +90,25 @@
   uint32_t pad2;
 };
 static_assert(sizeof(DTermAux) == 32, "DTermAux layout");
+
+struct alignas(16) DWalkRow {
+  uint64_t docids, fnorm;
+  uint64_t suffix;
+  uint64_t ub;
+  float    weight;
+  int32_t  fx_scale;
+  uint32_t flags;
+  uint32_t pad;
+  uint64_t u_after;
+  uint64_t look;
+  uint64_t cells, start;
+};
+static_assert(sizeof(DWalkRow) == 80, "DWalkRow layout");
+__host__ __device__ inline uint32_t walk_row_flags(uint32_t tab_slot, uint32_t fx_shift, uint32_t cache_slot, uint32_t cell_shift,
+                                                   uint32_t look_kind, uint32_t look_shift, bool must) {
+  return ((tab_slot & 0xFFFFu) < (uint32_t)kTabTerms ? (tab_slot & 0xFFFFu) : 7u) | (must ? 8u : 0u) | (fx_shift << 4) | (cache_slot << 8) |
+         ((cell_shift & 31u) << 16) | ((look_kind & 7u) << 24) | ((look_shift & 31u) << 27);
+}
 
 #ifndef NRT_MS_WIN_TILES
 #define NRT_MS_WIN_TILES 64
@@ -195,6 +223,7 @@
   uint64_t* item_hits;
   uint64_t* item_prof;
   const uint32_t* q_wins;
+  const DWalkRow* rows;
   uint32_t k_stride;
   uint32_t scatter;
   DHelp help;
diff --git a/nrtsearch_amd/csrc/planner.cpp b/nrtsearch_amd/csrc/planner.cpp
--- a/nrtsearch_amd/csrc/planner.cpp
+++ b/nrtsearch_amd/csrc/planner.cpp
@@ -376,7 +376,7 @@
     DQExpand& qx = qexpand[(size_t)qi];
     qx.term_begin = (uint32_t)pc.qterms.size();
     qx.by_weight = route != kRouteScan ? 1u : 0u;
-    qx.pad = 0;
+    qx.cache_off = 0;
     const uint32_t* cnt_of[kMaxTerms];
     bool req_of[kMaxTerms];
     uint32_t n_live = 0;
@@ -516,6 +516,7 @@
     for (QS& qs : pc.qs) qs.term_begin += dterm_base;
     for (int qi = chunk_begin(t); qi < chunk_begin(t + 1); ++qi) {
       cache_base[(size_t)qi] += c_base;
+      hp.qexpand[(size_t)qi].cache_off = cache_base[(size_t)qi];
       hp.qexpand[(size_t)qi].term_begin += qterm_base;
       piece_of[(size_t)qi] = t;
       if (dterm_base)
diff --git a/nrtsearch_amd/csrc/runtime_internal.h b/nrtsearch_amd/csrc/runtime_internal.h
--- a/nrtsearch_amd/csrc/runtime_internal.h
+++ b/nrtsearch_amd/csrc/runtime_internal.h
@@ -41,6 +41,8 @@
 void launch_bm25_maxscore(hipStream_t stream, bool profile, bool packed, int shapes, const MsArgs& args, const MsArgs* args_d);
 #ifdef NRTGPU_DEV
 void launch_debug_wave_kth(hipStream_t stream, const uint64_t* keys, uint32_t n, uint32_t r, uint64_t* out);
+void launch_debug_walk_value(hipStream_t stream, float weight, const uint32_t* freq, const uint32_t* norm, const float* table, int fx_scale,
+                             uint32_t fx_shift, uint32_t n, uint64_t* out);
 #endif
 void launch_term_frontier(hipStream_t stream, const uint32_t* fnorm, const uint64_t* t_start, const uint32_t* t_count,
                           const uint64_t* t_look, const uint32_t* t_meta, const void* look_base, uint32_t n_terms, DTermAux* out);
diff --git a/nrtsearch_amd/csrc/search.cpp b/nrtsearch_amd/csrc/search.cpp
--- a/nrtsearch_amd/csrc/search.cpp
+++ b/nrtsearch_amd/csrc/search.cpp
@@ -81,7 +81,7 @@
   const size_t o_items = pc.take(n_items * sizeof(DItem));
   const size_t o_parts = pc.take(hp.parts.size() * sizeof(DPart));
   const size_t o_qterms = pc.take(hp.qterms.size() * sizeof(DQTerm));
-  const size_t o_qexp = pc.take(hp.qexpand.size() * sizeof(DQExpand));
+  const size_t o_qexp = pc.take(sizeof(DExpandHead) + hp.qexpand.size() * sizeof(DQExpand)) + sizeof(DExpandHead);
   const size_t o_qsb = pc.take(hp.qs_begin.size() * 4);
   const size_t o_caches = pc.take(hp.caches.size() * sizeof(float));
   const size_t o_lidx = pc.take(hp.list_idx.size() * 4);
@@ -148,6 +148,8 @@
   const size_t o_ocnt = wc.take((size_t)n_queries * 4);
   const size_t o_ohits = wc.take((size_t)n_queries * 8);
   const size_t o_terms = wc.take((size_t)hp.n_dterms * sizeof(DTerm));
+  const bool walk_rows = hp.n_ms_items != 0 && dev_env_int("NRTGPU_MS_WALK_ROWS", 1) != 0;
+  const size_t o_rows = wc.take(walk_rows ? (size_t)hp.n_dterms * sizeof(DWalkRow) : 0);
   const size_t o_ssum = wc.take((size_t)n_queries * hp.n_slices * 4), o_qprune = wc.take((size_t)n_queries * 4);
   const size_t o_hwin = wc.take(hp.n_ms_items * 4), o_hcnt = wc.take(hp.n_ms_items * 4), o_ht0 = wc.take(hp.n_ms_items * 8);
   const size_t o_hhead = wc.take((size_t)n_queries * 4), o_hnext = wc.take(n_help * 4), o_hoff = wc.take(4);
@@ -214,6 +216,14 @@
   ms_args.item_hits = (uint64_t*)(wb + o_ihits);
   ms_args.item_prof = profile ? (uint64_t*)(wb + o_prof) : nullptr;
   ms_args.q_wins = (const uint32_t*)(db + o_qwins);
+  ms_args.rows = walk_rows ? (const DWalkRow*)(wb + o_rows) : nullptr;
+  {
+    DExpandHead xh{};
+    xh.caches = (const float*)(db + o_caches);
+    xh.queries = (const DQuery*)(db + o_queries);
+    xh.rows = walk_rows ? (DWalkRow*)(wb + o_rows) : nullptr;
+    memcpy(hb + o_qexp - sizeof(DExpandHead), &xh, sizeof(xh));
+  }
   {
     const long forced = dev_env_int("NRTGPU_MS_SCATTER", -1);
     ms_args.scatter = forced >= 0 ? (forced != 0 ? 1u : 0u) : ((spec && hp.lsc->spec_scattered.load(std::memory_order_relaxed) != 0) ? 1u : 0u);
```

Measured after the change: 554,000, median of 6. +6.0%, better.
